# ZhicengShi/mclSTExp

Measured on AMD Instinct MI355X. Metric: training spots/sec (= steps/sec x global batch) at batch 128/GPU, 224px patches, 1000 genes, higher is better.
Workload: dtype bf16; 1 GPU; BASELINE configs[1]: train step, batch 128/GPU, 224x224 patches, 1000 genes, densenet121 image encoder; global_batch=128, parallelism=dp1, backbone_dtype=bf16, infonce=fused, infonce_effective=exact (fused from 1024 pairs), hip_graphs=True, optimizer=Adam(lr=1e-4, wd=1e-3) incl. 2x(65536,G) tables

## Files before the change

include/mclstexp_hip.h:

```cpp
#ifndef MCLSTEXP_HIP_H
#define MCLSTEXP_HIP_H

#include <stddef.h>
#include <stdint.h>

#ifdef __cplusplus
extern "C" {
#endif

#define MCL_ABI_VERSION 13

#define MCL_OK 0
#define MCL_EINVAL (-1)
#define MCL_EUNSUPPORTED (-2)
#define MCL_EWORKSPACE (-3)

typedef void* mcl_stream_t;

int mcl_abi_version(void);
const char* mcl_error_string(int code);

#define MCL_EPI_GELU 1
#define MCL_EPI_GELU_BWD 2
#define MCL_EPI_ACCUM 4
// ... 97 lines not shown

int64_t mcl_infonce_fused_workspace_bytes(int32_t R, int32_t C, int32_t dim);
int mcl_infonce_fused_lse(const void* a, int64_t lda, const void* b, int64_t ldb, int32_t R, int32_t C, int32_t dim,
                          int32_t diag_off, float inv_temp, float* lse, float* diag, void* workspace, int64_t ws_bytes,
                          mcl_stream_t stream);
int mcl_infonce_fused_grad(const void* a, int64_t lda, const void* b, int64_t ldb, int32_t R, int32_t C, int32_t dim,
                           int32_t diag_off, float inv_temp, const float* lse_a, const float* lse_b, float coef, float* dA,
                           void* workspace, int64_t ws_bytes, mcl_stream_t stream);
int mcl_cast_f32_to_bf16(const float* x, int64_t ldx, void* y, int64_t ldy, int64_t rows, int32_t cols,
                         mcl_stream_t stream);

int64_t mcl_gemm_bf16_workspace_floats(int32_t M, int64_t ldc, int32_t ksplit);
int mcl_gemm_bf16(const void* A, int64_t lda, int64_t sAb, const void* B, int64_t ldb, int64_t sBb, void* C, int64_t ldc,
                  int64_t sCb, int32_t M, int32_t N, int32_t K, int32_t batch, int32_t batch2, int64_t sAb2, int64_t sBb2,
                  int64_t sCb2, float alpha, int32_t flags,
                  const float* bias, const void* resid, int64_t ldr, int64_t sRb, const void* aux, int64_t ldaux,
                  void* pre_out, int64_t ldp, int32_t ksplit, float* workspace, int32_t accumulate, mcl_stream_t stream);
int mcl_ln_bf16_fwd(const void* x, int64_t ldx, const float* gamma, const float* beta, void* y, int64_t ldy, float* mean,
                    float* rstd, int64_t rows, int32_t D, float eps, mcl_stream_t stream);
int64_t mcl_colred_workspace_floats(int64_t rows, int32_t D);
int mcl_ln_bf16_bwd(const void* dy, int64_t lddy, const void* x, int64_t ldx, const float* gamma, const float* mean,
                    const float* rstd, const void* dx_add, int64_t ldadd, void* dx, int64_t lddx, float* workspace,
                    float* dgamma, float* dbeta, int32_t accumulate, int64_t rows, int32_t D, mcl_stream_t stream);
int mcl_colsum_bf16(const void* x, int64_t ldx, int64_t rows, int32_t D, float* workspace, float* out, int32_t accumulate,
                    mcl_stream_t stream);
int mcl_softmax_bf16_fwd(void* s, int64_t ld, int64_t rows, int32_t n, mcl_stream_t stream);
int mcl_softmax_bf16_bwd(const void* P, void* dP, int64_t ld, int64_t rows, int32_t n, float scale, mcl_stream_t stream);
int mcl_vit_attn_fwd(const void* qkv, void* o, float* lse, int32_t B, int32_t T, int32_t heads, float scale, mcl_stream_t stream);
int mcl_vit_attn_bwd(const void* qkv, const void* o, const void* dout, const float* lse, float* dsum, void* dqkv, int32_t B,
                     int32_t T, int32_t heads, float scale, mcl_stream_t stream);
int mcl_vit_patchify_tokens(const float* img, int64_t sb, int64_t sc, int64_t sy, int64_t sx, int32_t B, int32_t H, int32_t W,
                            int32_t p, void* out, int32_t lead_zero_row, int32_t out_f32, mcl_stream_t stream);
int mcl_vit_cls_row(const float* cls, const float* pos, void* x, int32_t B, int32_t T, int32_t D, int32_t dtype,
                    mcl_stream_t stream);
int mcl_vit_assemble_f32(const float* tok, const float* cls, const float* pos, float* x, int32_t B, int32_t T, int32_t D,
                         mcl_stream_t stream);
int mcl_vit_tokens_extract(const void* dx, void* dtok, int32_t B, int32_t T, int32_t D, int32_t dtype, mcl_stream_t stream);
int mcl_vit_token_mean_fwd(const void* x, float* feat, int32_t B, int32_t T, int32_t D, int32_t dtype, mcl_stream_t stream);
int mcl_vit_token_mean_bwd(const float* dfeat, void* dx, int32_t B, int32_t T, int32_t D, int32_t dtype, mcl_stream_t stream);
int mcl_vit_pos_grad(const void* dx, float* dpos, float* dcls, int32_t B, int32_t T, int32_t D, int32_t dtype,
                     int32_t accumulate, mcl_stream_t stream);
int mcl_vit_zero_cls_rows(void* dx, int32_t B, int32_t T, int32_t D, int32_t dtype, mcl_stream_t stream);
int mcl_strided4_f32(const float* src, int32_t n0, int32_t n1, int32_t n2, int32_t n3, int64_t a0, int64_t a1, int64_t a2,
                     int64_t a3, void* dst, int64_t d0, int64_t d1, int64_t d2, int64_t d3, int32_t dst_dtype, int32_t accumulate,
                     mcl_stream_t stream);
int mcl_copy_rows(const void* src, int64_t ld_src_bytes, void* dst, int64_t ld_dst_bytes, int64_t rows, int64_t row_bytes,
                  mcl_stream_t stream);
int mcl_weight_rot180(const void* w, void* wf, int32_t Co, int32_t k, int32_t Ci, int32_t dtype, mcl_stream_t stream);
int mcl_vit_patchify(const float* img, int64_t sb, int64_t sc, int64_t sy, int64_t sx, int32_t B, int32_t H, int32_t W,
                     int32_t p, void* out_bf16, mcl_stream_t stream);

int mcl_quant_e4m3_rows(const float* x, int64_t ldx, int32_t rows, int32_t cols, void* q, int64_t ldq, void* scale,
                        int64_t ld_scale, void* deq_bf16, int64_t ldd, mcl_stream_t stream);
int mcl_dequant_e4m3_rows(const void* q, int64_t ldq, const void* scale, int64_t ld_scale, int32_t rows, int32_t cols,
                          void* deq_bf16, int64_t ldd, mcl_stream_t stream);
int64_t mcl_infonce_fp8_workspace_bytes(int32_t R, int32_t C);
int mcl_infonce_fp8_lse(const void* a8, int64_t lda, const void* scale_a, int64_t ld_sa, const void* b8, int64_t ldb,
                        const void* scale_b, int64_t ld_sb, int32_t R, int32_t C, int32_t dim, float inv_temp, float* lse,
                        void* workspace, int64_t ws_bytes, mcl_stream_t stream);
int mcl_infonce_rowdot_bf16(const void* a, int64_t lda, const void* b, int64_t ldb, int32_t R, int32_t C, int32_t dim,
                            int32_t diag_off, float inv_temp, float* diag, mcl_stream_t stream);

int64_t mcl_bn_workspace_floats(int64_t S, int32_t C, int32_t dtype);
int mcl_bn_stats(const void* x, int64_t ld, int64_t S, int32_t C, int32_t dtype, void* copy_out, int64_t ld_out,
                 float* workspace, float eps, float* mean, float* var, float* rstd, mcl_stream_t stream);
int mcl_bn_act_fwd(const void* x, int64_t ldx, int64_t S, int32_t C, int32_t dtype, const float* gamma,
                   const float* beta, const float* mean, const float* rstd, int32_t relu, void* y, int64_t ldy,
                   mcl_stream_t stream);
int mcl_bn_act_bwd(const void* dy, int64_t lddy, const void* x, int64_t ldx, int64_t S, int32_t C, int32_t dtype,
                   const float* gamma, const float* beta, const float* mean, const float* rstd, int32_t relu,
                   float* workspace, float* dgamma, float* dbeta, int32_t accumulate_params, void* dx, int64_t lddx,
                   int32_t accumulate, mcl_stream_t stream);

int64_t mcl_dense_conv1x1_workspace_floats(int64_t S);
int mcl_dense_conv1x1_fwd(const void* x, int64_t ldx, int64_t S, int32_t K, const float* gamma, const float* beta,
                          const float* mean, const float* rstd, const void* W, void* z, int64_t ldz, float* workspace,
                          float eps, float* zmean, float* zvar, float* zrstd, mcl_stream_t stream);

int64_t mcl_dense_conv3x3_workspace_floats(int64_t S);
int mcl_dense_conv3x3_fwd(const void* z, int64_t S, int32_t H, int32_t W, const float* gamma, const float* beta,
                          const float* mean, const float* rstd, const void* W2, void* out, int64_t ldo,
                          float* workspace, float eps, float* ymean, float* yvar, float* yrstd, mcl_stream_t stream);

int64_t mcl_dense_conv3x3_wrw_workspace_floats(int64_t S);
int mcl_dense_conv3x3_wrw_det(const void* dy, int64_t lddy, const void* z, int64_t S, int32_t H, int32_t W,
                              const float* gamma, const float* beta, const float* mean, const float* rstd,
                              float* workspace, float* dW, int32_t accumulate_w, mcl_stream_t stream);

int64_t mcl_dense_bn1_bwd_workspace_floats(int64_t S, int32_t C);
int mcl_dense_bn1_bwd(const void* dz, const void* W1, int32_t C, const void* x, int64_t ldx, int64_t S,
                      const float* gamma, const float* beta, const float* mean, const float* rstd, float* workspace,
                      float* dgamma, float* dbeta, int32_t accumulate_params, void* gbuf, int64_t ldg,
                      mcl_stream_t stream);

int mcl_dense_bn1_dx_window(const void* dz, const void* W1, int32_t C, int32_t c0, int32_t nc, const void* x, int64_t ldx,
                            int64_t S, const float* gamma, const float* beta, const float* mean, const float* rstd,
                            const float* coef, void* gbuf, int64_t ldg, mcl_stream_t stream);
int mcl_dense_bn1_dx_pair(const void* dzA, const void* W1A, int32_t ldwA, const float* gammaA, const float* betaA,
                          const float* coefA, const void* dzB, const void* W1B, const float* gammaB, const float* betaB,
                          const float* coefB, int32_t C, const void* x, int64_t ldx, int64_t S, const float* mean,
                          const float* rstd, void* gbuf, int64_t ldg, mcl_stream_t stream);

int64_t mcl_wrw_workspace_floats(int64_t S, int32_t M, int32_t N);
int mcl_dense_bn1_wrw(const void* dz, const void* W1, int32_t C, const void* x, int64_t ldx, int64_t S,
                      const float* gamma, const float* beta, const float* mean, const float* rstd, float* workspace,
                      float* dW, int32_t accumulate_w, float* dgamma, float* dbeta, int32_t accumulate_params,
                      float* coef_out, mcl_stream_t stream);
int mcl_dense_bn1_dx(const void* dz, const void* W1, int32_t C, const void* x, int64_t ldx, int64_t S,
                     const float* gamma, const float* beta, const float* mean, const float* rstd, const float* coef,
                     void* gbuf, int64_t ldg, mcl_stream_t stream);
int mcl_dense_bn1_dx_sums(const void* dz, const void* W1, int32_t C, const void* x, int64_t ldx, int64_t S,
                          const float* gamma, const float* beta, const float* mean, const float* rstd, float* workspace,
                          float* dgamma, float* dbeta, int32_t accumulate_params, float* kprev, int32_t have_prev, void* gbuf,
                          int64_t ldg, mcl_stream_t stream);
int mcl_dense_bn1_fix(const void* x, int64_t ldx, void* gbuf, int64_t ldg, int64_t S, int32_t c0, int32_t nc,
                      const float* mean, const float* rstd, const float* kacc, mcl_stream_t stream);
int mcl_conv1x1_wrw_det(const void* dz, int64_t ldz, const void* a, int64_t lda, const float* gamma, const float* beta,
                        const float* mean, const float* rstd, float* workspace, float* dW, int32_t accumulate_w,
                        int64_t S, int32_t M, int32_t N, mcl_stream_t stream);

int64_t mcl_dense_conv3x3_bwd_workspace_floats(int64_t S);
int mcl_dense_conv3x3_bwd(const void* dy, int64_t lddy, int64_t S, int32_t H, int32_t W, const void* W2, const void* z,
                          const float* gamma, const float* beta, const float* mean, const float* rstd, float* workspace,
                          float* dgamma, float* dbeta, int32_t accumulate_params, void* g2, void* dz, mcl_stream_t stream);
int mcl_dense_conv3x3_bwd_fix(const void* dy, int64_t lddy, int64_t S, int32_t H, int32_t W, const void* W2, const void* z,
                              const float* gamma, const float* beta, const float* mean, const float* rstd, float* workspace,
                              float* dgamma, float* dbeta, int32_t accumulate_params, void* g2, void* dz, const void* xfix,
                              int64_t ldxf, const float* fmean, const float* frstd, const float* fk, void* dyc,
                              mcl_stream_t stream);

int mcl_avgpool2_nhwc_bf16(const void* x, void* y, int32_t N, int32_t H, int32_t W, int32_t C, int32_t backward,
                           mcl_stream_t stream);
int mcl_maxpool3s2_nhwc_bf16_fwd(const void* x, void* y, void* idx, int32_t N, int32_t H, int32_t W, int32_t C,
                                 mcl_stream_t stream);
int mcl_maxpool3s2_nhwc_bf16_bwd(const void* idx, const void* dy, void* dx, int32_t N, int32_t H, int32_t W, int32_t C,
                                 mcl_stream_t stream);
int mcl_maxpool3s2_nhwc_bf16_bwd_ld(const void* idx, const void* dy, int64_t lddy, void* dx, int32_t N, int32_t H, int32_t W,
                                    int32_t C, mcl_stream_t stream);

int mcl_bn_act_avgpool_fwd(const void* x, int64_t ldx, int32_t N, int32_t H, int32_t W, int32_t C, const float* gamma,
                           const float* beta, const float* mean, const float* rstd, void* y, int64_t ldy,
                           mcl_stream_t stream);
int mcl_bn_act_avgpool_bwd(const void* dp, int64_t lddp, const void* x, int64_t ldx, int32_t N, int32_t H, int32_t W,
                           int32_t C, const float* gamma, const float* beta, const float* mean, const float* rstd,
                           float* workspace, float* dgamma, float* dbeta, int32_t accumulate_params, void* dx,
                           int64_t lddx, mcl_stream_t stream);
int64_t mcl_conv0_workspace_floats(int32_t N, int32_t H, int32_t W);
int mcl_conv0_fwd(const void* x, int32_t N, int32_t H, int32_t W, const void* Wt, void* y, float* workspace, float eps,
                  float* mean, float* var, float* rstd, mcl_stream_t stream);
int64_t mcl_conv0_wrw_workspace_floats(int32_t N, int32_t H, int32_t W);
int mcl_conv0_wrw(const void* x, int32_t N, int32_t H, int32_t W, const void* dy, float* workspace, float* dW,
                  int32_t accumulate_w, mcl_stream_t stream);

int mcl_bn_act_maxpool_fwd(const void* x, int32_t N, int32_t H, int32_t W, int32_t C, const float* gamma,
                           const float* beta, const float* mean, const float* rstd, void* y, void* idx,
                           mcl_stream_t stream);
int mcl_accum_into_f32(float* dst, const void* src, int64_t n, int32_t src_dtype, mcl_stream_t stream);

int mcl_bn_gap_fwd(const void* x, int64_t ldx, int32_t B, int32_t HW, int32_t C, const float* gamma, const float* beta,
                   const float* mean, const float* rstd, float* out, float* xmean, mcl_stream_t stream);
int mcl_bn_gap_bwd(const float* g, const float* xmean, const void* x, int64_t ldx, int32_t B, int32_t HW, int32_t C,
                   const float* gamma, const float* mean, const float* rstd, float* coef, float* dgamma, float* dbeta,
                   int32_t accumulate_params, void* dx, int64_t lddx, mcl_stream_t stream);
int mcl_bn_eval_rstd(int32_t n, const float* const* running_var, float* const* rstd_out, const int32_t* C, const float* eps,
                     mcl_stream_t stream);
int mcl_bn_running_update(int32_t n, float* const* running_mean, float* const* running_var, const float* const* mean,
                          const float* const* var, int64_t* const* num_batches_tracked, const int32_t* C,
                          const float* factor, const float* momentum, mcl_stream_t stream);
int mcl_image_to_bf16_nhwc(const float* x, int64_t sb, int64_t sc, int64_t sy, int64_t sx, int32_t B, int32_t C, int32_t H,
                           int32_t W, void* y, mcl_stream_t stream);
int mcl_fill_zero(void* p, int64_t bytes, mcl_stream_t stream);
int mcl_dropout_fwd(const float* x, float* y, void* mask, int64_t n, float p, uint64_t seed, mcl_stream_t stream);
int mcl_dropout_bwd(const float* dy, const void* mask, float* dx, int64_t n, float p, mcl_stream_t stream);
int mcl_gelu_f32(const float* x, const float* dy, float* out, int64_t n, mcl_stream_t stream);
int mcl_add_f32(const float* a, const float* b, float* y, int64_t n, mcl_stream_t stream);
int mcl_stamp(void* buf, int32_t idx, mcl_stream_t stream);
int mcl_scale2_f32(const float* a, int64_t na, const float* b, int64_t nb, const float* s, float* ya, float* yb,
                   mcl_stream_t stream);

int mcl_im2col_nhwc(const void* x, int64_t ldx, int32_t N, int32_t H, int32_t W, int32_t C, int32_t KH, int32_t KW,
                    int32_t stride, int32_t pad, int32_t dtype, void* cols, mcl_stream_t stream);
int mcl_col2im_nhwc(const void* dcols, int32_t N, int32_t H, int32_t W, int32_t C, int32_t KH, int32_t KW, int32_t stride,
                    int32_t pad, int32_t dtype, void* dx, int64_t lddx, int32_t accumulate, mcl_stream_t stream);
int mcl_maxpool3s2_nhwc_fwd_any(const void* x, void* y, void* idx, int32_t N, int32_t H, int32_t W, int32_t C, int32_t dtype,
                                mcl_stream_t stream);
int mcl_maxpool3s2_nhwc_bwd_any(const void* idx, const void* dy, void* dx, int32_t N, int32_t H, int32_t W, int32_t C,
                                int32_t dtype, mcl_stream_t stream);
int mcl_avgpool2_nhwc_any(const void* x, void* y, int32_t N, int32_t H, int32_t W, int32_t C, int32_t backward, int32_t dtype,
                          mcl_stream_t stream);
int mcl_gap_nhwc_fwd(const void* x, int64_t ldx, int32_t B, int32_t HW, int32_t C, int32_t dtype, float* out,
                     mcl_stream_t stream);
int mcl_gap_nhwc_bwd(const float* g, int32_t B, int32_t HW, int32_t C, int32_t dtype, void* dx, mcl_stream_t stream);
int mcl_add_relu(const void* a, const void* b, void* y, int64_t n, int32_t backward, int32_t dtype, mcl_stream_t stream);

int mcl_dense_block_pack_w1(const void* const* w1_ptrs, void* const* out_ptrs, int32_t L, int32_t C0, mcl_stream_t stream);
int64_t mcl_dense_block_fwd_workspace_bytes(int32_t B, int32_t L);
int mcl_dense_block_fwd(void* buf, int32_t B, int32_t H, int32_t W, int32_t Ct, int32_t C0, int32_t L,
                        const void* const* layer_ptrs, float eps1, float eps2, float* mean, float* var, float* rstd,
                        void* workspace, int32_t* err_flag, uint32_t max_spins, void* stamps, mcl_stream_t stream);

int mcl_dense_block_pack_bwd(const void* const* w1_ptrs, const void* const* w2_ptrs, void* const* w1t_ptrs,
                             void* const* w2t_ptrs, int32_t L, int32_t C0, mcl_stream_t stream);
int64_t mcl_dense_block_bwd_workspace_bytes(int32_t B, int32_t L);
int mcl_dense_block_bwd(const void* buf, void* gbuf, int32_t B, int32_t H, int32_t W, int32_t Ct, int32_t C0, int32_t L,
                        const void* const* layer_ptrs, const float* mean, const float* rstd, void* workspace,
                        int32_t* err_flag, uint32_t max_spins, void* stamps, mcl_stream_t stream);

int mcl_adam_step(float* p, const float* g, float* m, float* v, int64_t n, double lr, double beta1, double beta2,
                  double eps, double weight_decay, double bc1, double bc2, mcl_stream_t stream);
int mcl_adam_table_step(float* p, float* m, float* v, int32_t n_rows, int32_t cols, const int32_t* row_slot,
                        const float* row_grad, int64_t ld_rg, double lr, double beta1, double beta2, double eps,
                        double weight_decay, double bc1, double bc2, mcl_stream_t stream);
// ... 286 lines not shown
```

mclstexp_amd/_lib.py:

```python
from __future__ import annotations

import ctypes as C
import os
from typing import Optional

import torch

_HERE = os.path.dirname(os.path.abspath(__file__))
LIB_PATH = os.environ.get("MCL_LIB_PATH") or os.path.join(_HERE, "libmclstexp_hip.so")
ABI_VERSION = 13

_lib: Optional[C.CDLL] = None

c_f = C.c_float
c_d = C.c_double
c_i = C.c_int32
c_l = C.c_int64
c_p = C.c_void_p


class c_s(C.c_void_p):
    """mcl_stream_t: the trailing stream slot of an entry point.  ``call`` fills it in with torch's current stream."""


# ... 63 lines not shown
    "mcl_infonce_dlogits": [c_p, c_l, c_p, c_p, c_i, c_i, c_i, c_i, c_f, c_p, c_l, c_s],
    "mcl_infonce_fused_workspace_bytes": [c_i, c_i, c_i],
    "mcl_infonce_fused_lse": [c_p, c_l, c_p, c_l, c_i, c_i, c_i, c_i, c_f, c_p, c_p, c_p, c_l, c_s],
    "mcl_infonce_fused_grad": [c_p, c_l, c_p, c_l, c_i, c_i, c_i, c_i, c_f, c_p, c_p, c_f, c_p, c_p, c_l, c_s],
    "mcl_cast_f32_to_bf16": [c_p, c_l, c_p, c_l, c_l, c_i, c_s],
    "mcl_infonce_loss_mean": [c_p, c_l, c_p, c_p, c_i, c_f, c_p, c_s],
    "mcl_adam_step_dev_shadow": [c_p, c_p, c_p, c_p, c_l, c_p, c_p, c_s],
    "mcl_bn_gap_fwd": [c_p, c_l, c_i, c_i, c_i, c_p, c_p, c_p, c_p, c_p, c_p, c_s],
    "mcl_bn_gap_bwd": [c_p, c_p, c_p, c_l, c_i, c_i, c_i, c_p, c_p, c_p, c_p, c_p, c_p, c_i, c_p, c_l, c_s],
    "mcl_bn_running_update": [c_i, c_p, c_p, c_p, c_p, c_p, c_p, c_p, c_p, c_s],
    "mcl_bn_eval_rstd": [c_i, c_p, c_p, c_p, c_p, c_s],
    "mcl_image_to_bf16_nhwc": [c_p, c_l, c_l, c_l, c_l, c_i, c_i, c_i, c_i, c_p, c_s],
    "mcl_fill_zero": [c_p, c_l, c_s],
    "mcl_stamp": [c_p, c_i, c_s],
    "mcl_dropout_fwd": [c_p, c_p, c_p, c_l, c_f, C.c_uint64, c_s],
    "mcl_dropout_bwd": [c_p, c_p, c_p, c_l, c_f, c_s],
    "mcl_gelu_f32": [c_p, c_p, c_p, c_l, c_s],
    "mcl_add_f32": [c_p, c_p, c_p, c_l, c_s],
    "mcl_im2col_nhwc": [c_p, c_l, c_i, c_i, c_i, c_i, c_i, c_i, c_i, c_i, c_i, c_p, c_s],
    "mcl_col2im_nhwc": [c_p, c_i, c_i, c_i, c_i, c_i, c_i, c_i, c_i, c_i, c_p, c_l, c_i, c_s],
    "mcl_maxpool3s2_nhwc_fwd_any": [c_p, c_p, c_p, c_i, c_i, c_i, c_i, c_i, c_s],
    "mcl_maxpool3s2_nhwc_bwd_any": [c_p, c_p, c_p, c_i, c_i, c_i, c_i, c_i, c_s],
    "mcl_avgpool2_nhwc_any": [c_p, c_p, c_i, c_i, c_i, c_i, c_i, c_i, c_s],
    "mcl_gap_nhwc_fwd": [c_p, c_l, c_i, c_i, c_i, c_i, c_p, c_s],
    "mcl_gap_nhwc_bwd": [c_p, c_i, c_i, c_i, c_i, c_p, c_s],
    "mcl_add_relu": [c_p, c_p, c_p, c_l, c_i, c_i, c_s],
    "mcl_scale2_f32": [c_p, c_l, c_p, c_l, c_p, c_p, c_p, c_s],
    "mcl_maxpool3s2_nhwc_bf16_bwd_ld": [c_p, c_p, c_l, c_p, c_i, c_i, c_i, c_i, c_s],
    "mcl_gemm_bf16_workspace_floats": [c_i, c_l, c_i],
    "mcl_gemm_bf16": [c_p, c_l, c_l, c_p, c_l, c_l, c_p, c_l, c_l, c_i, c_i, c_i, c_i, c_i, c_l, c_l, c_l, c_f, c_i, c_p,
                      c_p, c_l, c_l, c_p, c_l, c_p, c_l, c_i, c_p, c_i, c_s],
    "mcl_ln_bf16_fwd": [c_p, c_l, c_p, c_p, c_p, c_l, c_p, c_p, c_l, c_i, c_f, c_s],
    "mcl_colred_workspace_floats": [c_l, c_i],
    "mcl_ln_bf16_bwd": [c_p, c_l, c_p, c_l, c_p, c_p, c_p, c_p, c_l, c_p, c_l, c_p, c_p, c_p, c_i, c_l, c_i, c_s],
    "mcl_colsum_bf16": [c_p, c_l, c_l, c_i, c_p, c_p, c_i, c_s],
    "mcl_softmax_bf16_fwd": [c_p, c_l, c_l, c_i, c_s],
    "mcl_softmax_bf16_bwd": [c_p, c_p, c_l, c_l, c_i, c_f, c_s],
    "mcl_vit_patchify": [c_p, c_l, c_l, c_l, c_l, c_i, c_i, c_i, c_i, c_p, c_s],
    "mcl_vit_patchify_tokens": [c_p, c_l, c_l, c_l, c_l, c_i, c_i, c_i, c_i, c_p, c_i, c_i, c_s],
    "mcl_vit_cls_row": [c_p, c_p, c_p, c_i, c_i, c_i, c_i, c_s],
    "mcl_vit_assemble_f32": [c_p, c_p, c_p, c_p, c_i, c_i, c_i, c_s],
    "mcl_vit_tokens_extract": [c_p, c_p, c_i, c_i, c_i, c_i, c_s],
    "mcl_vit_token_mean_fwd": [c_p, c_p, c_i, c_i, c_i, c_i, c_s],
    "mcl_vit_token_mean_bwd": [c_p, c_p, c_i, c_i, c_i, c_i, c_s],
    "mcl_vit_pos_grad": [c_p, c_p, c_p, c_i, c_i, c_i, c_i, c_i, c_s],
    "mcl_vit_zero_cls_rows": [c_p, c_i, c_i, c_i, c_i, c_s],
    "mcl_strided4_f32": [c_p, c_i, c_i, c_i, c_i, c_l, c_l, c_l, c_l, c_p, c_l, c_l, c_l, c_l, c_i, c_i, c_s],
    "mcl_copy_rows": [c_p, c_l, c_p, c_l, c_l, c_l, c_s],
    "mcl_weight_rot180": [c_p, c_p, c_i, c_i, c_i, c_i, c_s],
    "mcl_vit_attn_fwd": [c_p, c_p, c_p, c_i, c_i, c_i, c_f, c_s],
    "mcl_vit_attn_bwd": [c_p, c_p, c_p, c_p, c_p, c_p, c_i, c_i, c_i, c_f, c_s],
    "mcl_quant_e4m3_rows": [c_p, c_l, c_i, c_i, c_p, c_l, c_p, c_l, c_p, c_l, c_s],
    "mcl_dequant_e4m3_rows": [c_p, c_l, c_p, c_l, c_i, c_i, c_p, c_l, c_s],
    "mcl_infonce_fp8_workspace_bytes": [c_i, c_i],
    "mcl_infonce_fp8_lse": [c_p, c_l, c_p, c_l, c_p, c_l, c_p, c_l, c_i, c_i, c_i, c_f, c_p, c_p, c_l, c_s],
    "mcl_infonce_rowdot_bf16": [c_p, c_l, c_p, c_l, c_i, c_i, c_i, c_i, c_f, c_p, c_s],
    "mcl_bn_workspace_floats": [c_l, c_i, c_i],
    "mcl_bn_stats": [c_p, c_l, c_l, c_i, c_i, c_p, c_l, c_p, c_f, c_p, c_p, c_p, c_s],
    "mcl_bn_act_fwd": [c_p, c_l, c_l, c_i, c_i, c_p, c_p, c_p, c_p, c_i, c_p, c_l, c_s],
    "mcl_bn_act_bwd": [c_p, c_l, c_p, c_l, c_l, c_i, c_i, c_p, c_p, c_p, c_p, c_i, c_p, c_p, c_p, c_i, c_p, c_l, c_i, c_s],
    "mcl_dense_conv1x1_workspace_floats": [c_l],
    "mcl_dense_conv1x1_fwd": [c_p, c_l, c_l, c_i, c_p, c_p, c_p, c_p, c_p, c_p, c_l, c_p, c_f, c_p, c_p, c_p, c_s],
    "mcl_dense_conv3x3_workspace_floats": [c_l],
    "mcl_dense_bn1_bwd_workspace_floats": [c_l, c_i],
    "mcl_dense_conv3x3_bwd_workspace_floats": [c_l],
    "mcl_avgpool2_nhwc_bf16": [c_p, c_p, c_i, c_i, c_i, c_i, c_i, c_s],
    "mcl_maxpool3s2_nhwc_bf16_fwd": [c_p, c_p, c_p, c_i, c_i, c_i, c_i, c_s],
    "mcl_maxpool3s2_nhwc_bf16_bwd": [c_p, c_p, c_p, c_i, c_i, c_i, c_i, c_s],
    "mcl_dense_conv3x3_bwd": [c_p, c_l, c_l, c_i, c_i, c_p, c_p, c_p, c_p, c_p, c_p, c_p, c_p, c_p, c_i, c_p, c_p, c_s],
    "mcl_dense_conv3x3_bwd_fix": [c_p, c_l, c_l, c_i, c_i, c_p, c_p, c_p, c_p, c_p, c_p, c_p, c_p, c_p, c_i, c_p, c_p, c_p,
                                  c_l, c_p, c_p, c_p, c_p, c_s],
    "mcl_dense_bn1_bwd": [c_p, c_p, c_i, c_p, c_l, c_l, c_p, c_p, c_p, c_p, c_p, c_p, c_p, c_i, c_p, c_l, c_s],
    "mcl_dense_conv3x3_wrw_workspace_floats": [c_l],
    "mcl_dense_conv3x3_wrw_det": [c_p, c_l, c_p, c_l, c_i, c_i, c_p, c_p, c_p, c_p, c_p, c_p, c_i, c_s],
    "mcl_wrw_workspace_floats": [c_l, c_i, c_i],
    "mcl_dense_bn1_wrw": [c_p, c_p, c_i, c_p, c_l, c_l, c_p, c_p, c_p, c_p, c_p, c_p, c_i, c_p, c_p, c_i, c_p, c_s],
    "mcl_dense_bn1_dx_window": [c_p, c_p, c_i, c_i, c_i, c_p, c_l, c_l, c_p, c_p, c_p, c_p, c_p, c_p, c_l, c_s],
    "mcl_dense_bn1_dx_pair": [c_p, c_p, c_i, c_p, c_p, c_p, c_p, c_p, c_p, c_p, c_p, c_i, c_p, c_l, c_l, c_p, c_p, c_p, c_l, c_s],
    "mcl_dense_bn1_dx": [c_p, c_p, c_i, c_p, c_l, c_l, c_p, c_p, c_p, c_p, c_p, c_p, c_l, c_s],
    "mcl_dense_bn1_dx_sums": [c_p, c_p, c_i, c_p, c_l, c_l, c_p, c_p, c_p, c_p, c_p, c_p, c_p, c_i, c_p, c_i, c_p, c_l, c_s],
    "mcl_dense_bn1_fix": [c_p, c_l, c_p, c_l, c_l, c_i, c_i, c_p, c_p, c_p, c_s],
    "mcl_conv1x1_wrw_det": [c_p, c_l, c_p, c_l, c_p, c_p, c_p, c_p, c_p, c_p, c_i, c_l, c_i, c_i, c_s],
    "mcl_dense_conv3x3_fwd": [c_p, c_l, c_i, c_i, c_p, c_p, c_p, c_p, c_p, c_p, c_l, c_p, c_f, c_p, c_p, c_p, c_s],
    "mcl_accum_into_f32": [c_p, c_p, c_l, c_i, c_s],
    "mcl_adam_step": [c_p, c_p, c_p, c_p, c_l, c_d, c_d, c_d, c_d, c_d, c_d, c_d, c_s],
    "mcl_adam_table_step": [c_p, c_p, c_p, c_i, c_i, c_p, c_p, c_l, c_d, c_d, c_d, c_d, c_d, c_d, c_d, c_s],
    "mcl_adam_consts_update": [c_p, c_p, c_p, c_s],
    "mcl_adam_step_dev": [c_p, c_p, c_p, c_p, c_l, c_p, c_s],
    "mcl_adam_table_step_dev": [c_p, c_p, c_p, c_i, c_i, c_p, c_p, c_l, c_p, c_s],
    "mcl_row_slot_update": [c_p, c_p, c_i, c_i, c_s],
    "mcl_dense_block_fwd_workspace_bytes": [c_i, c_i],
    "mcl_dense_block_pack_w1": [c_p, c_p, c_i, c_i, c_s],
    "mcl_dense_block_pack_bwd": [c_p, c_p, c_p, c_p, c_i, c_i, c_s],
    "mcl_dense_block_bwd_workspace_bytes": [c_i, c_i],
    "mcl_dense_block_bwd": [c_p, c_p, c_i, c_i, c_i, c_i, c_i, c_i, c_p, c_p, c_p, c_p, c_p, C.c_uint32, c_p, c_s],
    "mcl_dense_block_fwd": [c_p, c_i, c_i, c_i, c_i, c_i, c_i, c_p, c_f, c_f, c_p, c_p, c_p, c_p, c_p, C.c_uint32, c_p, c_s],
    "mcl_adam_consts_update_hist": [c_p, c_p, c_p, c_p, c_i, c_s],
    "mcl_adam_table_lazy": [c_p, c_p, c_p, c_p, c_p, c_p, c_p, c_p, c_i, c_i, c_p, c_p, c_p, c_i, c_p, c_p, c_l, c_p, c_p, c_i,
                            c_s],
    "mcl_bn_act_avgpool_fwd": [c_p, c_l, c_i, c_i, c_i, c_i, c_p, c_p, c_p, c_p, c_p, c_l, c_s],
    "mcl_bn_act_avgpool_bwd": [c_p, c_l, c_p, c_l, c_i, c_i, c_i, c_i, c_p, c_p, c_p, c_p, c_p, c_p, c_p, c_i, c_p, c_l,
                               c_s],
    "mcl_conv0_workspace_floats": [c_i, c_i, c_i],
    "mcl_conv0_fwd": [c_p, c_i, c_i, c_i, c_p, c_p, c_p, c_f, c_p, c_p, c_p, c_s],
    "mcl_conv0_wrw_workspace_floats": [c_i, c_i, c_i],
    "mcl_conv0_wrw": [c_p, c_i, c_i, c_i, c_p, c_p, c_p, c_i, c_s],
    "mcl_bn_act_maxpool_fwd": [c_p, c_i, c_i, c_i, c_i, c_p, c_p, c_p, c_p, c_p, c_p, c_s],
    "mcl_patch_gather": [c_p, c_i, c_i, c_p, c_i, c_i, c_p, c_f, c_p, c_p, c_s],
    "mcl_her2st_train_patches": [c_p, c_i, c_i, c_p, c_i, c_i, c_p, c_f, c_p, c_p, c_s],
    "mcl_log_library_size_normalize": [c_p, c_l, c_p, c_l, c_i, c_i, c_f, c_s],
    "mcl_l2_normalize_rows": [c_p, c_l, c_p, c_l, c_i, c_i, c_s],
    "mcl_topk_rows_max_k": [],
    "mcl_topk_rows": [c_p, c_l, c_i, c_i, c_i, c_p, c_p, c_s],
    "mcl_topk_rows_indexed": [c_p, c_l, c_p, c_l, c_i, c_i, c_i, c_p, c_p, c_p, c_s],
    "mcl_knn_weighted_average": [c_p, c_l, c_p, c_l, c_p, c_l, c_p, c_i, c_i, c_i, c_i, c_i, c_p, c_p, c_s],
    "mcl_expr_metrics": [c_p, c_l, c_i, c_p, c_l, c_i, c_p, c_i, c_i, c_i, c_p, c_p, c_p, c_p, c_p, c_s],
    "mcl_pearson_pvalue": [c_p, c_p, c_i, c_i, c_p, c_p, c_s],
    "mcl_gene_rank": [c_p, c_p, c_i, c_i, c_i, c_p, c_p, c_p, c_p, c_p, c_p, c_s],
    "mcl_knn_combine": [c_p, c_l, c_p, c_l, c_p, c_l, c_p, c_i, c_i, c_i, c_i, c_i, c_p, c_p, c_s],
    "mcl_cell_pearson": [c_p, c_l, c_i, c_p, c_l, c_i, c_l, c_i, c_p, c_s],
    "mcl_bleep_summary": [c_p, c_l, c_i, c_p, c_i, c_i, c_i, c_p, c_p, c_p, c_i, c_p, c_p, c_p, c_p, c_p, c_s],
    "mcl_corr_from_gram": [c_p, c_i, c_p, c_s],
    "mcl_pca_gram": [c_p, c_l, c_i, c_p, c_i, c_i, c_i, c_p, c_p, c_p, c_s],
    "mcl_pca_project": [c_p, c_l, c_i, c_p, c_i, c_i, c_i, c_i, c_p, c_p, c_p, c_p, c_p, c_p, c_p, c_s],
    "mcl_kmeans": [c_p, c_l, c_p, c_i, c_l, c_i, c_p, c_i, c_i, c_p, C.c_uint64, c_i, c_d, c_i, c_p, c_p, c_p, c_p, c_p, c_p,
                   c_p, c_p, c_p, c_p, c_p, c_s],
    "mcl_cluster_scores": [c_p, c_p, c_p, c_i, c_i, c_p, c_s],
    "mcl_hvg_stats": [c_p, c_p, c_p, c_p, c_p, c_i, c_p, c_i, c_i, c_i, c_i, c_p, c_p, c_p, c_p, c_p, c_p, c_p, c_p, c_p, c_s],
    "mcl_hvg_pool": [c_p, c_i, c_i, c_p, c_i, c_p, c_p, c_s],
    "mcl_expression_matrices": [c_p, c_p, c_p, c_p, c_p, c_i, c_p, c_i, c_i, c_i, c_f, c_p, c_s],
    "mcl_harmony_workspace_doubles": [c_i, c_i, c_i, c_i],
    "mcl_harmony_normalize": [c_p, c_l, c_i, c_i, c_i, c_i, c_p, c_p, c_s],
    "mcl_harmony_centroids": [c_p, c_p, c_p, c_i, c_i, c_i, c_i, c_i, c_p, c_p, c_s],
    "mcl_harmony_dist": [c_p, c_p, c_i, c_i, c_i, c_i, c_p, c_s],
    "mcl_harmony_softmax": [c_p, c_i, c_i, c_d, c_i, c_p, c_s],
    "mcl_harmony_moments": [c_p, c_p, c_i, c_i, c_i, c_p, c_p, c_p, c_s],
    "mcl_harmony_update_block": [c_p, c_p, c_p, c_p, c_i, c_i, c_i, c_i, c_i, c_i, c_p, c_p, c_p, c_p, c_s],
    "mcl_harmony_objective": [c_p, c_p, c_p, c_p, c_p, c_p, c_i, c_i, c_i, c_d, c_p, c_p, c_s],
    "mcl_harmony_ridge": [c_p, c_p, c_p, c_i, c_i, c_i, c_p, c_s],
    "mcl_harmony_apply": [c_p, c_p, c_p, c_p, c_i, c_i, c_i, c_i, c_p, c_s],
    "mcl_harmony_lloyd": [c_p, c_i, c_i, c_i, c_p, c_i, c_p, c_p, c_p, c_p, c_p, c_s],
    "mcl_tsne_workspace_doubles": [c_i, c_i],
    "mcl_tsne_affinities": [c_p, c_l, c_i, c_i, c_p, c_p, c_i, c_i, c_i, c_i, c_l, c_d, c_i, c_p, c_p, c_p, c_s],
    "mcl_tsne_gradient": [c_p, c_p, c_p, c_p, c_i, c_i, c_i, c_i, c_l, c_p, c_i, c_p, c_p, c_p, c_s],
    "mcl_tsne_update": [c_p, c_p, c_i, c_i, c_i, c_i, c_p, c_p, c_p, c_p, c_p, c_s],
    "mcl_knn_workspace_bytes": [c_i, c_i],
    "mcl_knn_exact": [c_p, c_l, c_i, c_i, c_p, c_i, c_i, c_i, c_i, c_i, c_p, c_p, c_s],
    "mcl_knn_smooth": [c_p, c_p, c_i, c_i, c_i, c_i, c_i, c_p, c_p, c_p, c_s],
    "mcl_knn_connectivities": [c_p, c_p, c_p, c_p, c_p, c_i, c_i, c_i, c_i, c_i, c_d, c_i, c_p, c_p, c_p, c_p, c_l, c_p, c_p,
                               c_s],
    "mcl_umap_workspace_bytes": [c_l, c_i],
    "mcl_umap_prepare": [c_p, c_p, c_p, c_i, c_l, c_l, c_i, c_i, c_p, c_p, c_s],
    "mcl_umap_init": [c_i, c_p, c_l, c_i, c_i, c_p, c_i, c_i, c_i, c_i, C.c_uint64, c_p, c_s],
    "mcl_umap_epochs": [c_i, c_i, c_p, c_p, c_p, c_p, c_p, c_i, c_i, c_i, c_i, c_l, c_i, c_d, c_d, c_d, c_d, c_i, C.c_uint64,
                        c_p, c_p, c_p, c_p, c_s],
    "mcl_leiden_workspace_bytes": [c_l, c_l, c_i, c_i],
    "mcl_leiden_init": [c_p, c_p, c_p, c_p, c_p, c_i, c_i, c_i, c_l, c_d, c_p, c_p, c_p, c_p],
    "mcl_leiden_move_sweeps": [c_i, c_i, c_i, c_i, c_i, c_p, c_p, c_p, c_p, c_i, c_i, c_i, c_l, c_d, c_p, c_p],
    "mcl_leiden_refine_rounds": [c_i, c_i, c_i, c_i, c_i, c_i, c_p, c_p, c_p, c_p, c_i, c_i, c_i, c_l, c_d, c_p, c_p],
    "mcl_leiden_aggregate": [c_i, c_i, c_i, c_p, c_p, c_p, c_p, c_i, c_i, c_i, c_l, c_d, c_p, c_p],
    "mcl_leiden_finish": [c_i, c_i, c_p, c_p, c_p, c_p, c_p, c_i, c_i, c_i, c_l, c_p, c_p, c_p, c_p, c_p],
    "mcl_sym_eig_workspace_bytes": [c_i, c_i, c_l, c_i],
    "mcl_sym_eig_top": [c_p, c_p, c_p, c_i, c_i, c_l, c_i, c_i, c_p, c_p, c_p, c_p, c_p, c_p],
    "mcl_marker_workspace_bytes": [c_l, c_l, c_i, c_i],
    "mcl_marker_stats": [c_p, c_l, c_i, c_p, c_p, c_p, c_i, c_l, c_i, c_i, c_i, c_l, c_p, c_p, c_p, c_p, c_p, c_p, c_p, c_p,
                         c_p, c_p, c_p, c_p, c_p],
# ... 197 lines not shown
```

mclstexp_amd/csrc/dense_bwd.hip:

```cpp
#include "common.h"
#include <stdlib.h>

namespace {

constexpr int TN = 128, TK = 128;

__device__ __forceinline__ uint4 keep4(bool keep, const uint4 v) {
  return make_uint4(keep ? v.x : 0u, keep ? v.y : 0u, keep ? v.z : 0u, keep ? v.w : 0u);
}

template <int MODE, int TMv>
__global__ __launch_bounds__(256, (TMv == 64 && MODE != 2 ? 3 : 2)) void bn1_bwd_kernel(const bf16_t* __restrict__ dz, const bf16_t* __restrict__ W1,
                                                         int K , int ldw ,
                                                         const bf16_t* __restrict__ x, long long ldx, long long S,
                                                         const float* __restrict__ gamma,
                                                         const float* __restrict__ beta,
                                                         const float* __restrict__ mean,
                                                         const float* __restrict__ rstd,
                                                         const float* __restrict__ coef ,
                                                         bf16_t* gbuf, long long ldg,
                                                         float2* __restrict__ partial , int nrt) {
  __shared__ __attribute__((aligned(16))) unsigned char lds[TK * 256 + TMv * 256 + 2048];
  const int tid = threadIdx.x, lane = tid & 63, wave = tid >> 6;
  const int h = lane >> 5, l31 = lane & 31;
// ... 404 lines not shown
  for (int o = 32; o > 0; o >>= 1) {
    a += __shfl_xor(a, o, 64);
    b += __shfl_xor(b, o, 64);
  }
  if (lane == 0) {
    red[0][wave] = a;
    red[1][wave] = b;
  }
  __syncthreads();
  if (threadIdx.x != 0) return;
  a = (red[0][0] + red[0][1]) + (red[0][2] + red[0][3]);
  b = (red[1][0] + red[1][1]) + (red[1][2] + red[1][3]);
  if (accumulate_params) {
    dbeta[c] += (float)a;
    dgamma[c] += (float)b;
  } else {
    dbeta[c] = (float)a;
    dgamma[c] = (float)b;
  }
  if (kacc != nullptr) {
    const double scv = (double)gamma[c] * (double)rstd[c];
    kacc[2 * c] = (float)(scv * a / (double)S);
    kacc[2 * c + 1] = (float)(scv * b / (double)S);
    return;
  }
  coef[2 * c] = (float)(a / (double)S);
  coef[2 * c + 1] = (float)(b / (double)S);
}

__global__ __launch_bounds__(256) void bn1_fix_kernel(const bf16_t* __restrict__ x, long long ldx, bf16_t* __restrict__ gbuf,
                                                      long long ldg, long long S, int c0, int nc,
                                                      const float* __restrict__ mean, const float* __restrict__ rstd,
                                                      const float* __restrict__ kacc) {
  const int cpr = nc >> 3;
  const long long n = S * cpr;
  const long long i0 = (long long)blockIdx.x * 256 + threadIdx.x, istride = (long long)gridDim.x * 256;
  const bool fixed = (istride % cpr) == 0;
  uint4 xv = make_uint4(0u, 0u, 0u, 0u), gv = xv;
  if (i0 < n) {
    const long long row = i0 / cpr;
    const int c = c0 + (int)(i0 - row * cpr) * 8;
    xv = *reinterpret_cast<const uint4*>(x + row * ldx + c);
    gv = *reinterpret_cast<const uint4*>(gbuf + row * ldg + c);
  }
  float kav[8], kbv[8];
  auto consts = [&](int c) {
#pragma unroll
    for (int e = 0; e < 8; ++e) {
      const float k1 = kacc[2 * (c + e)], k2 = kacc[2 * (c + e) + 1];
      kav[e] = k2 * rstd[c + e];
      kbv[e] = fmaf(-kav[e], mean[c + e], k1);
    }
  };
  if (i0 < n) consts(c0 + (int)(i0 % cpr) * 8);
  for (long long i = i0; i < n; i += istride) {
    const long long row = i / cpr;
    const int c = c0 + (int)(i - row * cpr) * 8;
    if (i != i0) {
      xv = *reinterpret_cast<const uint4*>(x + row * ldx + c);
      gv = *reinterpret_cast<const uint4*>(gbuf + row * ldg + c);
      if (!fixed) consts(c);
    }
    const unsigned xw[4] = {xv.x, xv.y, xv.z, xv.w};
    unsigned gw[4] = {gv.x, gv.y, gv.z, gv.w};
#pragma unroll
    for (int u = 0; u < 4; ++u) {
      float o[2];
#pragma unroll
      for (int e = 0; e < 2; ++e) {
        const float ka = kav[2 * u + e], kb = kbv[2 * u + e];
        const float xf = e ? __uint_as_float(xw[u] & 0xFFFF0000u) : __uint_as_float(xw[u] << 16);
        const float gf = e ? __uint_as_float(gw[u] & 0xFFFF0000u) : __uint_as_float(gw[u] << 16);
        o[e] = gf - fmaf(ka, xf, kb);
      }
      const f32x2 pv = {o[0], o[1]};
      gw[u] = __builtin_bit_cast(unsigned, __builtin_convertvector(pv, bf16x2_t));
    }
    *reinterpret_cast<uint4*>(gbuf + row * ldg + c) = make_uint4(gw[0], gw[1], gw[2], gw[3]);
  }
}

constexpr int C3I = 128, C3O = 32, T3B = 128;

__global__ __launch_bounds__(256, 1) void conv3x3_bwd_kernel(const bf16_t* __restrict__ dy, long long lddy, long long S,
                                                             int H, int W, const bf16_t* __restrict__ W2,
                                                             const bf16_t* __restrict__ z,
                                                             const float* __restrict__ gamma,
                                                             const float* __restrict__ beta,
                                                             const float* __restrict__ mean,
                                                             const float* __restrict__ rstd, bf16_t* __restrict__ g2,
                                                             float2* __restrict__ partial, int ntile,
                                                             const bf16_t* __restrict__ xfix, long long ldxf,
                                                             const float* __restrict__ fmean,
                                                             const float* __restrict__ frstd,
                                                             const float* __restrict__ fk, bf16_t* __restrict__ dyc) {
  extern __shared__ __attribute__((aligned(16))) unsigned char lds[];
  const int tid = threadIdx.x, lane = tid & 63, wave = tid >> 6;
  const int h = lane >> 5, l31 = lane & 31;
  const int nrow = T3B + 2 * W + 2;
  bf16_t* zt = reinterpret_cast<bf16_t*>(lds);
  unsigned char* slab = lds + T3B * 256;
  const int zero_off = T3B * 256 + nrow * 64;
  const int Si = (int)S;

  uint4 zr[8];
  auto load_z_tile = [&](int tile) {
    const int p0 = tile * T3B;
#pragma unroll
    for (int i = 0; i < 8; ++i) {
      const int p = p0 + (tid >> 4) + 16 * i;
      zr[i] = p < Si ? *reinterpret_cast<const uint4*>(z + (long long)p * C3I + (tid & 15) * 8) : make_uint4(0u, 0u, 0u, 0u);
    }
  };
  if ((int)blockIdx.x < ntile) load_z_tile(blockIdx.x);
  bf16x8 breg[18];
#pragma unroll
  for (int i = 0; i < 18; ++i) {
    const int tap = i >> 1, co0 = 16 * (i & 1) + 8 * h;
#pragma unroll
    for (int j = 0; j < 8; ++j)
      breg[i][j] = (short)W2[((long long)(co0 + j) * 9 + tap) * C3I + 32 * wave + l31];
  }
  const int c = 32 * wave + l31;
  const float mu = mean[c], rs = rstd[c];
  const float sc = gamma[c] * rs, sh = fmaf(-mu, sc, beta[c]);
  int abase[18];
#pragma unroll
  for (int i = 0; i < 18; ++i) {
    const int tap = i >> 1, ky = tap / 3, kx = tap % 3;
    const int row = l31 + (2 - ky) * W + (2 - kx);
    abase[i] = T3B * 256 + row * 64 + (((2 * (i & 1) + h) ^ ((row >> 2) & 3)) << 4);
  }
  if (tid < 4) *reinterpret_cast<uint4*>(lds + zero_off + tid * 16) = make_uint4(0u, 0u, 0u, 0u);
  float fka[8], fkb[8];
  if (xfix != nullptr) {
#pragma unroll
    for (int e = 0; e < 8; ++e) {
      const int cf = (tid & 3) * 8 + e;
      const float k1 = fk[2 * cf], k2 = fk[2 * cf + 1];
      fka[e] = k2 * frstd[cf];
      fkb[e] = fmaf(-fka[e], fmean[cf], k1);
    }
  }

  for (int tile = blockIdx.x; tile < ntile; tile += gridDim.x) {
    const int p0 = tile * T3B;
    if (tile != (int)blockIdx.x) load_z_tile(tile);
    __syncthreads();
    for (int q = tid; q < nrow * 4; q += 256) {
      const int j = q >> 2, ch = q & 3;
      const int p = p0 - (W + 1) + j;
      uint4 v = make_uint4(0u, 0u, 0u, 0u);
      if (p >= 0 && p < Si) {
        v = *reinterpret_cast<const uint4*>(dy + (long long)p * lddy + ch * 8);
        if (xfix != nullptr) {
          const uint4 xv = *reinterpret_cast<const uint4*>(xfix + (long long)p * ldxf + ch * 8);
          const unsigned xw[4] = {xv.x, xv.y, xv.z, xv.w};
          unsigned gw[4] = {v.x, v.y, v.z, v.w};
#pragma unroll
          for (int u = 0; u < 4; ++u) {
            const float o_lo = __uint_as_float(gw[u] << 16) - fmaf(fka[2 * u], __uint_as_float(xw[u] << 16), fkb[2 * u]);
            const float o_hi = __uint_as_float(gw[u] & 0xFFFF0000u) -
                               fmaf(fka[2 * u + 1], __uint_as_float(xw[u] & 0xFFFF0000u), fkb[2 * u + 1]);
            const f32x2 pv = {o_lo, o_hi};
            gw[u] = __builtin_bit_cast(unsigned, __builtin_convertvector(pv, bf16x2_t));
          }
          v = make_uint4(gw[0], gw[1], gw[2], gw[3]);
          if (dyc != nullptr && j >= W + 1 && j < W + 1 + T3B) *reinterpret_cast<uint4*>(dyc + (long long)p * C3O + ch * 8) = v;
        }
      }
      *reinterpret_cast<uint4*>(slab + j * 64 + ((ch ^ ((j >> 2) & 3)) << 4)) = v;
    }
#pragma unroll
    for (int i = 0; i < 8; ++i)
      *reinterpret_cast<uint4*>(zt + ((tid >> 4) + 16 * i) * C3I + (tid & 15) * 8) = zr[i];
    unsigned vmask[4];
#pragma unroll
    for (int mb = 0; mb < 4; ++mb) {
      const int p = p0 + mb * 32 + l31;
      const int x = p % W, y = (p / W) % H;
      unsigned m = 0;
      if (p < Si) {
#pragma unroll
        for (int ky = 0; ky < 3; ++ky)
#pragma unroll
          for (int kx = 0; kx < 3; ++kx) {
            const int yy = y + 1 - ky, xx = x + 1 - kx;
            if (yy >= 0 && yy < H && xx >= 0 && xx < W) m |= 1u << (ky * 3 + kx);
          }
      }
      vmask[mb] = m;
    }
    f32x16 acc[4];
#pragma unroll
    for (int mb = 0; mb < 4; ++mb)
#pragma unroll
      for (int r = 0; r < 16; ++r) acc[mb][r] = 0.0f;
    __syncthreads();

#pragma unroll
    for (int i = 0; i < 18; ++i) {
#pragma unroll
      for (int mb = 0; mb < 4; ++mb) {
        const int off = ((vmask[mb] >> (i >> 1)) & 1u) ? abase[i] + mb * 2048 : zero_off;
        const bf16x8 a = *reinterpret_cast<const bf16x8*>(lds + off);
        acc[mb] = __builtin_amdgcn_mfma_f32_32x32x16_bf16(a, breg[i], acc[mb], 0, 0, 0);
      }
    }
    const int nvalid = min(T3B, Si - p0);
    float s1 = 0.0f, s2 = 0.0f;
#pragma unroll
    for (int mb = 0; mb < 4; ++mb)
#pragma unroll
      for (int r = 0; r < 16; ++r) {
        const int px = mb * 32 + (r & 3) + 8 * (r >> 2) + 4 * h;
        const float zv = bf2f(zt[px * C3I + c]);
        const float gi = fmaf(zv, sc, sh) > 0.0f ? acc[mb][r] : 0.0f;
        const bf16_t gb = f2bf(gi);
        if (px < nvalid) {
          const float gr_ = bf2f(gb);
          s1 += gr_;
          s2 = fmaf(gr_, (zv - mu) * rs, s2);
        }
        zt[px * C3I + c] = gb;
      }
    s1 += __shfl_xor(s1, 32, 64);
    s2 += __shfl_xor(s2, 32, 64);
    if (h == 0) partial[(long long)c * ntile + tile] = make_float2(s1, s2);
    __syncthreads();
#pragma unroll
    for (int i = 0; i < 8; ++i) {
      const int r = (tid >> 4) + 16 * i;
      const int p = p0 + r;
      if (p < Si)
        *reinterpret_cast<uint4*>(g2 + (long long)p * C3I + (tid & 15) * 8) =
            *reinterpret_cast<const uint4*>(zt + r * C3I + (tid & 15) * 8);
    }
  }
}

constexpr int BR_NWAVE = 8;
constexpr int BR_SLOT = 34 * 64;
constexpr int BR_RING = 4 * BR_SLOT;

__device__ __forceinline__ void br_swap8(unsigned (&w)[8]) {
#pragma unroll
  for (int g = 0; g < 2; ++g)
#pragma unroll
    for (int d = 0; d < 2; ++d) {
      const u32x2 r = __builtin_amdgcn_permlane32_swap(w[4 * g + d], w[4 * g + 2 + d], false, false);
      w[4 * g + d] = r[0];
      w[4 * g + 2 + d] = r[1];
    }
}

template <bool K0, bool K2>
__device__ __forceinline__ void br_row_mfma(const unsigned char* __restrict__ ring, int jo, const int (&foff)[3][2],
                                            const bf16x8 (&breg)[18], f32x16& acc) {
// ... 326 lines not shown
  if (nb > 2048) nb = 2048;
  hipLaunchKernelGGL(bn1_fix_kernel, dim3((int)nb), dim3(256), 0, mcl_stream(stream), (const bf16_t*)x, (long long)ldx,
                     (bf16_t*)gbuf, (long long)ldg, (long long)S, c0, nc, mean, rstd, kacc);
  MCL_CHECK_LAUNCH();
  return MCL_OK;
}

namespace {
int bn1_dx_impl(const void* dz, const void* W1, int32_t C, int32_t ldw, const void* x, int64_t ldx, int64_t S, const float* gamma,
                const float* beta, const float* mean, const float* rstd, const float* coef, void* gbuf, int64_t ldg,
                mcl_stream_t stream) {
  if (!dz || !W1 || !x || !gamma || !beta || !mean || !rstd || !coef || !gbuf || S <= 0 || C <= 0 || ldw < C) return MCL_EINVAL;
  if ((C % 8) || (ldw % 8) || (ldx % 8) || (ldg % 8) || (reinterpret_cast<uintptr_t>(dz) & 15u) ||
      (reinterpret_cast<uintptr_t>(W1) & 15u) || (reinterpret_cast<uintptr_t>(x) & 15u) ||
      (reinterpret_cast<uintptr_t>(gbuf) & 15u))
    return MCL_EUNSUPPORTED;
  const int nrt = (int)((S + 63) / 64), nct = (C + TN - 1) / TN;
  const int gcap = S >= 50000 ? 512 : 768;
  int gx = (gcap + nct - 1) / nct;
  if (gx > nrt) gx = nrt;
  hipLaunchKernelGGL((bn1_bwd_kernel<1, 64>), dim3(gx, nct), dim3(256), 0, mcl_stream(stream), (const bf16_t*)dz,
                     (const bf16_t*)W1, C, ldw, (const bf16_t*)x, (long long)ldx, (long long)S, gamma, beta, mean, rstd, coef,
                     (bf16_t*)gbuf, (long long)ldg, (float2*)nullptr, nrt);
  MCL_CHECK_LAUNCH();
  return MCL_OK;
}
}

extern "C" int mcl_dense_bn1_dx(const void* dz, const void* W1, int32_t C, const void* x, int64_t ldx, int64_t S,
                                const float* gamma, const float* beta, const float* mean, const float* rstd,
                                const float* coef, void* gbuf, int64_t ldg, mcl_stream_t stream) {
  MCL_CLEAR_ERROR();
  return bn1_dx_impl(dz, W1, C, C, x, ldx, S, gamma, beta, mean, rstd, coef, gbuf, ldg, stream);
}

extern "C" int mcl_dense_bn1_dx_window(const void* dz, const void* W1, int32_t C, int32_t c0, int32_t nc, const void* x,
                                       int64_t ldx, int64_t S, const float* gamma, const float* beta, const float* mean,
                                       const float* rstd, const float* coef, void* gbuf, int64_t ldg, mcl_stream_t stream) {
  MCL_CLEAR_ERROR();
  if (c0 < 0 || nc <= 0 || c0 + nc > C || (c0 % 8)) return MCL_EINVAL;
  if (!dz || !W1 || !x || !gamma || !beta || !mean || !rstd || !coef || !gbuf) return MCL_EINVAL;
  return bn1_dx_impl(dz, (const bf16_t*)W1 + c0, nc, C, (const bf16_t*)x + c0, ldx, S, gamma + c0, beta + c0, mean + c0, rstd + c0,
                     coef + 2 * c0, (bf16_t*)gbuf + c0, ldg, stream);
}

extern "C" int mcl_dense_bn1_dx_pair(const void* dzA, const void* W1A, int32_t ldwA, const float* gammaA, const float* betaA,
                                     const float* coefA, const void* dzB, const void* W1B, const float* gammaB,
                                     const float* betaB, const float* coefB, int32_t C, const void* x, int64_t ldx, int64_t S,
                                     const float* mean, const float* rstd, void* gbuf, int64_t ldg, mcl_stream_t stream) {
  MCL_CLEAR_ERROR();
  if (!dzA || !W1A || !gammaA || !betaA || !coefA || !dzB || !W1B || !gammaB || !betaB || !coefB || !x || !mean || !rstd || !gbuf ||
      S <= 0 || C <= 0 || ldwA < C)
    return MCL_EINVAL;
  if ((C % 8) || (ldwA % 8) || (ldx % 8) || (ldg % 8) || (reinterpret_cast<uintptr_t>(dzA) & 15u) ||
      (reinterpret_cast<uintptr_t>(dzB) & 15u) || (reinterpret_cast<uintptr_t>(W1A) & 15u) ||
      (reinterpret_cast<uintptr_t>(W1B) & 15u) || (reinterpret_cast<uintptr_t>(x) & 15u) ||
      (reinterpret_cast<uintptr_t>(gbuf) & 15u))
    return MCL_EUNSUPPORTED;
  static mcl_device_once attr_once;
  if (auto guard = attr_once.first())
    (void)hipFuncSetAttribute(reinterpret_cast<const void*>(bn1_dx_pair_kernel), hipFuncAttributeMaxDynamicSharedMemorySize,
                              (int)PAIR_LDS);
  const int nrt = (int)((S + 63) / 64), nct = (C + TN - 1) / TN;
  const int gcap = 512;
  int gx = (gcap + nct - 1) / nct;
  if (gx > nrt) gx = nrt;
  hipLaunchKernelGGL(bn1_dx_pair_kernel, dim3(gx, nct), dim3(256), PAIR_LDS, mcl_stream(stream), (const bf16_t*)dzA,
                     (const bf16_t*)W1A, ldwA, gammaA, betaA, coefA, (const bf16_t*)dzB, (const bf16_t*)W1B, gammaB, betaB, coefB, C,
                     (const bf16_t*)x, (long long)ldx, (long long)S, mean, rstd, (bf16_t*)gbuf, (long long)ldg, nrt);
  MCL_CHECK_LAUNCH();
  return MCL_OK;
}

extern "C" int64_t mcl_dense_conv3x3_bwd_workspace_floats(int64_t S) {
  if (S <= 0) return -1;
  const int64_t flat = (S + T3B - 1) / T3B, rows = S / 32 + 8;
  return (flat > rows ? flat : rows) * 2 * (int64_t)C3I + 2 * (int64_t)C3I;
}

namespace {
int conv3x3_bwd_impl(const void* dy, int64_t lddy, int64_t S, int32_t H, int32_t W, const void* W2, const void* z,
                     const float* gamma, const float* beta, const float* mean, const float* rstd, float* workspace,
                     float* dgamma, float* dbeta, int32_t accumulate_params, void* g2, void* dz, const void* xfix,
                     int64_t ldxf, const float* fmean, const float* frstd, const float* fk, void* dyc, mcl_stream_t stream) {
  MCL_CLEAR_ERROR();
  if (!dy || !W2 || !z || !gamma || !beta || !mean || !rstd || !workspace || !dgamma || !dbeta || !g2 || !dz || S <= 0 ||
      H <= 0 || W <= 0)
    return MCL_EINVAL;
  if ((S % ((int64_t)H * W)) || S > 0x7fff0000LL || W > 150 || (lddy % 8) || lddy < C3O ||
      (reinterpret_cast<uintptr_t>(dy) & 15u) || (reinterpret_cast<uintptr_t>(z) & 15u) ||
      (reinterpret_cast<uintptr_t>(g2) & 15u) || (reinterpret_cast<uintptr_t>(dz) & 15u))
    return MCL_EUNSUPPORTED;
  if (xfix != nullptr) {
    if (!fmean || !frstd || !fk || !dyc) return MCL_EINVAL;
    if (bwd_rows_applicable(S, H, W) || (ldxf % 8) || (reinterpret_cast<uintptr_t>(xfix) & 15u) ||
        (reinterpret_cast<uintptr_t>(dyc) & 15u))
      return MCL_EUNSUPPORTED;
  }
  hipStream_t st = mcl_stream(stream);
  float2* part = reinterpret_cast<float2*>(workspace);
  float* coef;
  if (bwd_rows_applicable(S, H, W)) {
    const BwdRowsPlan p = bwd_rows_plan(S, H, W);
    coef = workspace + (int64_t)p.nsu * 2 * C3I;
    static mcl_device_once attr_once;
    if (auto attr_guard = attr_once.first()) {
      (void)hipFuncSetAttribute(reinterpret_cast<const void*>(conv3x3_bwd_rows_kernel),
                                hipFuncAttributeMaxDynamicSharedMemorySize, 160 * 1024);
    }
    hipLaunchKernelGGL(conv3x3_bwd_rows_kernel, dim3(p.grid), dim3(64 * BR_NWAVE), (size_t)BR_NWAVE * BR_RING + 1024, st,
                       (const bf16_t*)dy, (long long)lddy, p.nimg, H, W, (const bf16_t*)W2, (const bf16_t*)z, gamma, beta,
                       mean, rstd, (bf16_t*)g2, part, p.nsu, p.rc, p.nchunk, p.nstrip);
    hipLaunchKernelGGL(bn1_bwd_finalize_kernel, dim3(C3I), dim3(256), 0, st, (const float2*)part, p.nsu, C3I,
                       (long long)S, dgamma, dbeta, coef, accumulate_params);
  } else {
    const int ntile = (int)((S + T3B - 1) / T3B);
    coef = workspace + (int64_t)ntile * 2 * C3I;
    const size_t lds_bytes = (size_t)T3B * 256 + (size_t)(T3B + 2 * W + 2) * 64 + 64;
    const int gcap = S >= 50000 ? 512 : 768;
    hipLaunchKernelGGL(conv3x3_bwd_kernel, dim3(ntile < gcap ? ntile : gcap), dim3(256), lds_bytes, st, (const bf16_t*)dy,
                       (long long)lddy, (long long)S, H, W, (const bf16_t*)W2, (const bf16_t*)z, gamma, beta, mean, rstd,
                       (bf16_t*)g2, part, ntile, (const bf16_t*)xfix, (long long)ldxf, fmean, frstd, fk, (bf16_t*)dyc);
    hipLaunchKernelGGL(bn1_bwd_finalize_kernel, dim3(C3I), dim3(256), 0, st, (const float2*)part, ntile, C3I,
                       (long long)S, dgamma, dbeta, coef, accumulate_params);
  }
  const long long n_chunks = S * (C3I / 8);
  long long blocks = (n_chunks + 255) / 256;
  if (blocks > 2048) blocks = 2048;
  hipLaunchKernelGGL(bn2_dz_kernel, dim3((unsigned)blocks), dim3(256), 0, st, (const bf16_t*)g2, (const bf16_t*)z,
                     n_chunks, gamma, mean, rstd, (const float*)coef, (bf16_t*)dz);
  MCL_CHECK_LAUNCH();
  return MCL_OK;
}
}

extern "C" int mcl_dense_conv3x3_bwd(const void* dy, int64_t lddy, int64_t S, int32_t H, int32_t W, const void* W2,
                                     const void* z, const float* gamma, const float* beta, const float* mean,
                                     const float* rstd, float* workspace, float* dgamma, float* dbeta,
                                     int32_t accumulate_params, void* g2, void* dz, mcl_stream_t stream) {
  return conv3x3_bwd_impl(dy, lddy, S, H, W, W2, z, gamma, beta, mean, rstd, workspace, dgamma, dbeta, accumulate_params, g2,
                          dz, nullptr, 0, nullptr, nullptr, nullptr, nullptr, stream);
}

extern "C" int mcl_dense_conv3x3_bwd_fix(const void* dy, int64_t lddy, int64_t S, int32_t H, int32_t W, const void* W2,
                                         const void* z, const float* gamma, const float* beta, const float* mean,
                                         const float* rstd, float* workspace, float* dgamma, float* dbeta,
                                         int32_t accumulate_params, void* g2, void* dz, const void* xfix, int64_t ldxf,
                                         const float* fmean, const float* frstd, const float* fk, void* dyc,
                                         mcl_stream_t stream) {
  if (!xfix) return MCL_EINVAL;
  return conv3x3_bwd_impl(dy, lddy, S, H, W, W2, z, gamma, beta, mean, rstd, workspace, dgamma, dbeta, accumulate_params, g2,
                          dz, xfix, ldxf, fmean, frstd, fk, dyc, stream);
}
```

mclstexp_amd/csrc/dense_conv.hip:

```cpp
#include "common.h"

namespace {

constexpr int BN = 128;
constexpr int BK = 64;

template <int WM, int RW = 64, int DEPTH = 1>
__global__ __launch_bounds__(128 * WM) void conv1x1_fwd_kernel(const bf16_t* __restrict__ x, long long ldx, long long S,
                                                               int K, const float* __restrict__ gamma,
                                                               const float* __restrict__ beta,
                                                               const float* __restrict__ mean,
                                                               const float* __restrict__ rstd,
                                                               const bf16_t* __restrict__ W, bf16_t* __restrict__ z,
                                                               long long ldz, float2* __restrict__ partial, int nblk) {
  constexpr int BM = RW * WM, NT = 128 * WM;
  constexpr int RI = RW / 32;
  constexpr int NA = (BM * 8) / NT;
  constexpr int A_B = BM * 128, B_B = BN * 128, STAGE_B = A_B + B_B;
  constexpr int NB = (BN * 8) / NT;
  constexpr int NBUF = DEPTH == 0 ? 1 : 2, NSET = DEPTH == 0 ? 1 : DEPTH;
  __shared__ __attribute__((aligned(16))) unsigned char lds[NBUF * STAGE_B + 2 * 1024 * 4];
  float* tab = reinterpret_cast<float*>(lds + NBUF * STAGE_B);

  const int tid = threadIdx.x, lane = tid & 63, wave = tid >> 6;
// ... 240 lines not shown
    red[0][wave] = sum;
    red[1][wave] = q;
  }
  __syncthreads();
  if (threadIdx.x != 0) return;
  sum = (red[0][0] + red[0][1]) + (red[0][2] + red[0][3]);
  q = (red[1][0] + red[1][1]) + (red[1][2] + red[1][3]);
  const double n = (double)S, m = sum / n;
  double v = (q - sum * sum / n) / n;
  if (v < 0.0) v = 0.0;
  mean[c] = (float)m;
  var[c] = (float)v;
  rstd[c] = (float)(1.0 / sqrt(v + (double)eps));
}

inline int pick_wm(long long S) { return S >= 32768 ? 2 : 1; }

}

extern "C" int64_t mcl_dense_conv1x1_workspace_floats(int64_t S) {
  if (S <= 0) return -1;
  const int bm = 64 * pick_wm(S);
  return ((S + bm - 1) / bm) * BN * 2;
}

extern "C" int mcl_dense_conv1x1_fwd(const void* x, int64_t ldx, int64_t S, int32_t K, const float* gamma,
                                     const float* beta, const float* mean, const float* rstd, const void* W, void* z,
                                     int64_t ldz, float* workspace, float eps, float* zmean, float* zvar,
                                     float* zrstd, mcl_stream_t stream) {
  MCL_CLEAR_ERROR();
  if (!x || !gamma || !beta || !mean || !rstd || !W || !z || !workspace || S <= 0 || K <= 0) return MCL_EINVAL;
  const bool want_stats = zmean || zvar || zrstd;
  if (want_stats && (!zmean || !zvar || !zrstd)) return MCL_EINVAL;
  if ((K % 8) || K > 1024 || (ldx % 8) || (ldz % 8) || ldz < BN || S * ldx * 2 >= 0xFFFFF000LL  ||
      (reinterpret_cast<uintptr_t>(x) & 15u) ||
      (reinterpret_cast<uintptr_t>(W) & 15u) || (reinterpret_cast<uintptr_t>(z) & 15u))
    return MCL_EUNSUPPORTED;
  const int wm = pick_wm(S);
  const int bm = 64 * wm;
  const int nblk = (int)((S + bm - 1) / bm);
  hipStream_t st = mcl_stream(stream);
  float2* part = reinterpret_cast<float2*>(workspace);
#define MCL_LAUNCH(WMV, RWV, DPV)                                                                                    \
  hipLaunchKernelGGL((conv1x1_fwd_kernel<WMV, RWV, DPV>), dim3(nblk), dim3(128 * WMV), 0, st, (const bf16_t*)x,      \
                     (long long)ldx, (long long)S, K, gamma, beta, mean, rstd, (const bf16_t*)W, (bf16_t*)z,          \
                     (long long)ldz, part, nblk)
  if (wm == 2) MCL_LAUNCH(2, 64, 0);
  else MCL_LAUNCH(2, 32, 4);
#undef MCL_LAUNCH
  if (want_stats)
    hipLaunchKernelGGL(tile_stats_finalize_kernel, dim3(BN), dim3(256), 0, st, (const float2*)part, nblk, BN,
                       (long long)S, bm, eps, zmean, zvar, zrstd);
  MCL_CHECK_LAUNCH();
  return MCL_OK;
}

constexpr int C3_IN = 128, C3_OUT = 32, T3 = 128;

constexpr int SLAB_NB = 8;
template <int NB>
__device__ __forceinline__ void stage_slab(unsigned char* lds, const bf16_t* __restrict__ z, int p0, long long S,
                                           int W, int nrow, int tid, const float (&sc)[8], const float (&sh)[8]) {
  const int cc = tid & 15;
  for (int jb = tid >> 4; jb < nrow; jb += 16 * NB) {
    uint4 v[NB];
    bool ok[NB];
#pragma unroll
    for (int i = 0; i < NB; ++i) {
      const int j = jb + 16 * i;
      const int p = p0 - (W + 1) + j;
      ok[i] = j < nrow && p >= 0 && p < (int)S;
      v[i] = ok[i] ? *reinterpret_cast<const uint4*>(z + (long long)p * C3_IN + cc * 8) : make_uint4(0u, 0u, 0u, 0u);
    }
#pragma unroll
    for (int i = 0; i < NB; ++i) {
      const int j = jb + 16 * i;
      if (j < nrow)
        *reinterpret_cast<uint4*>(lds + j * 256 + ((cc ^ (j & 15)) << 4)) =
            ok[i] ? bn_relu_chunk(v[i], sc, sh) : make_uint4(0u, 0u, 0u, 0u);
    }
  }
}

__global__ __launch_bounds__(256, 2) void conv3x3_fwd_kernel(const bf16_t* __restrict__ z, long long S, int H, int W,
                                                             const float* __restrict__ gamma,
                                                             const float* __restrict__ beta,
                                                             const float* __restrict__ mean,
                                                             const float* __restrict__ rstd,
                                                             const bf16_t* __restrict__ W2, bf16_t* __restrict__ out,
                                                             long long ldo, float2* __restrict__ partial, int ntile) {
  extern __shared__ __attribute__((aligned(16))) unsigned char lds[];
  const int tid = threadIdx.x, lane = tid & 63, wave = tid >> 6;
  const int h = lane >> 5, l31 = lane & 31;
  const int nrow = T3 + 2 * W + 2;
  unsigned char* zero_row = lds + nrow * 256;
  const int Si = (int)S;

  bf16x8 breg[18];
#pragma unroll
  for (int i = 0; i < 18; ++i) {
    const int kidx = 18 * wave + i;
    breg[i] = *reinterpret_cast<const bf16x8*>(W2 + ((long long)l31 * 9 + (kidx >> 3)) * C3_IN + 16 * (kidx & 7) + 8 * h);
  }
  float sc[8], sh[8];
  {
    const int cc = tid & 15;
#pragma unroll
    for (int i = 0; i < 8; ++i) {
      const int c = cc * 8 + i;
      sc[i] = gamma[c] * rstd[c];
      sh[i] = fmaf(-mean[c], sc[i], beta[c]);
    }
  }
  int abase[18], tapk[18];
#pragma unroll
  for (int i = 0; i < 18; ++i) {
    const int kidx = 18 * wave + i, tap = kidx >> 3, kk = kidx & 7;
    const int row = l31 + (tap / 3) * W + (tap % 3);
    abase[i] = row * 256 + (((2 * kk + h) ^ (row & 15)) << 4);
    tapk[i] = tap;
  }
  for (int tile = blockIdx.x; tile < ntile; tile += gridDim.x) {
  const int p0 = tile * T3;
  __syncthreads();

  stage_slab<SLAB_NB>(lds, z, p0, S, W, nrow, tid, sc, sh);
  if (tid < 16) *reinterpret_cast<uint4*>(zero_row + tid * 16) = make_uint4(0u, 0u, 0u, 0u);

  unsigned vmask[4];
#pragma unroll
  for (int mb = 0; mb < 4; ++mb) {
    const int p = p0 + mb * 32 + l31;
    const int x = p % W, y = (p / W) % H;
    unsigned m = 0;
    if (p < Si) {
#pragma unroll
      for (int ky = 0; ky < 3; ++ky)
#pragma unroll
        for (int kx = 0; kx < 3; ++kx) {
          const int yy = y + ky - 1, xx = x + kx - 1;
          if (yy >= 0 && yy < H && xx >= 0 && xx < W) m |= 1u << (ky * 3 + kx);
        }
    }
    vmask[mb] = m;
  }
  f32x16 acc[4];
#pragma unroll
  for (int mb = 0; mb < 4; ++mb)
#pragma unroll
    for (int r = 0; r < 16; ++r) acc[mb][r] = 0.0f;
  __syncthreads();

  const int zero_off = nrow * 256;
#pragma unroll
  for (int i = 0; i < 18; ++i) {
#pragma unroll
    for (int mb = 0; mb < 4; ++mb) {
      const int off = ((vmask[mb] >> tapk[i]) & 1u) ? abase[i] + mb * 8192 : zero_off;
      const bf16x8 a = *reinterpret_cast<const bf16x8*>(lds + off);
      acc[mb] = __builtin_amdgcn_mfma_f32_32x32x16_bf16(a, breg[i], acc[mb], 0, 0, 0);
    }
  }
  __syncthreads();
  float* red = reinterpret_cast<float*>(lds);
#pragma unroll
  for (int mb = 0; mb < 4; ++mb)
#pragma unroll
    for (int r = 0; r < 16; ++r) {
      const int px = mb * 32 + (r & 3) + 8 * (r >> 2) + 4 * h;
      red[(wave * T3 + px) * C3_OUT + l31] = acc[mb][r];
    }
  __syncthreads();
  const int px = tid >> 1, c0 = (tid & 1) * 16;
  const long long p = (long long)p0 + px;
  float v[16];
#pragma unroll
  for (int q = 0; q < 4; ++q) {
    float4 s = *reinterpret_cast<const float4*>(red + px * C3_OUT + c0 + 4 * q);
#pragma unroll
    for (int w = 1; w < 4; ++w) {
      const float4 t = *reinterpret_cast<const float4*>(red + (w * T3 + px) * C3_OUT + c0 + 4 * q);
      s.x += t.x; s.y += t.y; s.z += t.z; s.w += t.w;
    }
    v[4 * q] = s.x; v[4 * q + 1] = s.y; v[4 * q + 2] = s.z; v[4 * q + 3] = s.w;
  }
  unsigned pk[8];
#pragma unroll
  for (int q = 0; q < 8; ++q) pk[q] = pack_bf16(v[2 * q], v[2 * q + 1]);
  if (p < S) {
    *reinterpret_cast<uint4*>(out + p * ldo + c0) = make_uint4(pk[0], pk[1], pk[2], pk[3]);
    *reinterpret_cast<uint4*>(out + p * ldo + c0 + 8) = make_uint4(pk[4], pk[5], pk[6], pk[7]);
  }
  __syncthreads();
  float* rv = reinterpret_cast<float*>(lds);
  float* grp = rv + T3 * C3_OUT;
#pragma unroll
  for (int q = 0; q < 8; ++q) {
    rv[px * C3_OUT + c0 + 2 * q] = bf_lo(pk[q]);
    rv[px * C3_OUT + c0 + 2 * q + 1] = bf_hi(pk[q]);
  }
  __syncthreads();
  {
    const int c = tid & 31, g = tid >> 5;
    const float ks = rv[c];
    const int nvalid = min(T3, Si - p0);
    float s1 = 0.0f, s2 = 0.0f;
#pragma unroll
    for (int q = 0; q < 16; ++q) {
      const int pp = g * 16 + q;
      if (pp < nvalid) {
        const float dlt = rv[pp * C3_OUT + c] - ks;
        s1 += dlt;
        s2 = fmaf(dlt, dlt, s2);
      }
    }
    grp[(g * 32 + c) * 2] = s1;
    grp[(g * 32 + c) * 2 + 1] = s2;
    __syncthreads();
    if (tid < 32) {
      float a = 0.0f, b = 0.0f;
#pragma unroll
      for (int gg = 0; gg < 8; ++gg) {
        a += grp[(gg * 32 + tid) * 2];
        b += grp[(gg * 32 + tid) * 2 + 1];
      }
      const float n = (float)nvalid;
      partial[(long long)tid * ntile + tile] = make_float2(fmaf(n, rv[tid], a), b - a * a / n);
    }
  }
  }
}

extern "C" int64_t mcl_dense_conv3x3_workspace_floats(int64_t S) {
  if (S <= 0) return -1;
  const int64_t flat = ((S + T3 - 1) / T3) * C3_OUT * 2, rows = mcl_conv3x3_rows_workspace_floats(S);
  return flat > rows ? flat : rows;
}

extern "C" int mcl_dense_conv3x3_fwd(const void* z, int64_t S, int32_t H, int32_t W, const float* gamma,
                                     const float* beta, const float* mean, const float* rstd, const void* W2, void* out,
                                     int64_t ldo, float* workspace, float eps, float* ymean, float* yvar, float* yrstd,
                                     mcl_stream_t stream) {
  MCL_CLEAR_ERROR();
  if (!z || !gamma || !beta || !mean || !rstd || !W2 || !out || !workspace || S <= 0 || H <= 0 || W <= 0)
    return MCL_EINVAL;
  const bool want_stats = ymean || yvar || yrstd;
  if (want_stats && (!ymean || !yvar || !yrstd)) return MCL_EINVAL;
  if ((S % ((int64_t)H * W)) || S > 0x7fff0000LL || W > 150 || (ldo % 8) || ldo < C3_OUT || (reinterpret_cast<uintptr_t>(z) & 15u) ||
      (reinterpret_cast<uintptr_t>(W2) & 15u) || (reinterpret_cast<uintptr_t>(out) & 15u))
    return MCL_EUNSUPPORTED;
  if (mcl_conv3x3_rows_applicable(S, H, W)) {
    const int rc = mcl_launch_conv3x3_fwd_rows(z, S, H, W, gamma, beta, mean, rstd, W2, out, ldo, workspace, eps, ymean,
                                               yvar, yrstd, mcl_stream(stream));
    if (rc != 0) return rc;
    MCL_CHECK_LAUNCH();
    return MCL_OK;
  }
  const int ntile = (int)((S + T3 - 1) / T3);
  size_t lds_bytes = (size_t)(T3 + 2 * W + 2) * 256 + 256;
  if (lds_bytes < 4 * T3 * C3_OUT * 4) lds_bytes = 4 * T3 * C3_OUT * 4;
  hipStream_t st = mcl_stream(stream);
  static mcl_device_once attr_once;
  if (auto attr_guard = attr_once.first()) {
    (void)hipFuncSetAttribute(reinterpret_cast<const void*>(conv3x3_fwd_kernel),
                              hipFuncAttributeMaxDynamicSharedMemorySize, 112 * 1024);
  }
  float2* part = reinterpret_cast<float2*>(workspace);
  hipLaunchKernelGGL(conv3x3_fwd_kernel, dim3(ntile < 512 ? ntile : 512), dim3(256), lds_bytes, st, (const bf16_t*)z, (long long)S, H, W,
                     gamma, beta, mean, rstd, (const bf16_t*)W2, (bf16_t*)out, (long long)ldo, part, ntile);
  if (want_stats)
    hipLaunchKernelGGL(tile_stats_finalize_kernel, dim3(C3_OUT), dim3(256), 0, st, (const float2*)part, ntile,
                       C3_OUT, (long long)S, T3, eps, ymean, yvar, yrstd);
  MCL_CHECK_LAUNCH();
  return MCL_OK;
}

namespace {

__device__ __forceinline__ int w3k_swz(int row) { return ((row & 3) << 2) | ((row >> 2) & 3); }

constexpr int W3K_ROWS = T3 + 2;
constexpr int W3K_LDS = W3K_ROWS * 256 + 3 * T3 * 64;

__global__ __launch_bounds__(256, 2) void conv3x3_wrw_ky_kernel(const bf16_t* __restrict__ dy, long long lddy,
                                                                const bf16_t* __restrict__ z, long long S, int H, int W,
                                                                const float* __restrict__ gamma,
                                                                const float* __restrict__ beta,
                                                                const float* __restrict__ mean,
                                                                const float* __restrict__ rstd, int ntile, int G,
                                                                float* __restrict__ wpart) {
  __shared__ __attribute__((aligned(16))) unsigned char lds[W3K_LDS];
  const int tid = threadIdx.x, lane = tid & 63, wave = tid >> 6;
  const int h = lane >> 5, l31 = lane & 31;
  const int xcd = blockIdx.x & 7, slot = blockIdx.x >> 3;
  const int ky = slot % 3, g = (slot / 3) * 8 + xcd;
  if (g >= G) return;
  unsigned char* zt = lds;
  unsigned char* dyt = lds + W3K_ROWS * 256;
  const int Si = (int)S;

  const int cc = tid & 15, rz = tid >> 4;
  const int rd = tid >> 1, cd = (tid & 1) * 2;
  float sc[8], sh[8];
#pragma unroll
  for (int i = 0; i < 8; ++i) {
    const int c = cc * 8 + i;
    sc[i] = gamma[c] * rstd[c];
    sh[i] = fmaf(-mean[c], sc[i], beta[c]);
  }
  f32x16 acc[3];
#pragma unroll
  for (int b = 0; b < 3; ++b)
#pragma unroll
    for (int r = 0; r < 16; ++r) acc[b][r] = 0.0f;

  const int i15 = lane & 15, q = i15 >> 2, jj = i15 & 3;
  const int half16 = 16 * ((lane >> 4) & 1);
  const int byte = (jj & 1) * 8;
  int bz_lo[3], bz_hi[3];
#pragma unroll
  for (int kx = 0; kx < 3; ++kx) {
    const int chunk = wave * 4 + ((half16 + jj * 4) >> 3);
    const int r0 = 8 * h + q + kx, r1 = r0 + 4;
    bz_lo[kx] = r0 * 256 + ((chunk ^ w3k_swz(r0)) << 4) + byte;
    bz_hi[kx] = r1 * 256 + ((chunk ^ w3k_swz(r1)) << 4) + byte;
  }
  const int dchunk = (half16 + jj * 4) >> 3;

  auto fetch = [&](uint4 (&zv)[9], uint4 (&dv)[2], int tile) {
    const int p0 = tile * T3;
    const int qs = p0 + (ky - 1) * W - 1;
#pragma unroll
    for (int i = 0; i < 9; ++i) {
      const int j = rz + 16 * i;
      const int p = qs + j;
      zv[i] = (tile < ntile && j < W3K_ROWS && p >= 0 && p < Si)
                  ? *reinterpret_cast<const uint4*>(z + (long long)p * C3_IN + cc * 8)
                  : make_uint4(0u, 0u, 0u, 0u);
    }
    const int p = p0 + rd;
#pragma unroll
    for (int u = 0; u < 2; ++u)
      dv[u] = (tile < ntile && p < Si) ? *reinterpret_cast<const uint4*>(dy + (long long)p * lddy + (cd + u) * 8)
                                       : make_uint4(0u, 0u, 0u, 0u);
  };
  auto stage = [&](const uint4 (&zv)[9], const uint4 (&dv)[2], int tile) {
    const int p0 = tile * T3;
    const int qs = p0 + (ky - 1) * W - 1;
#pragma unroll
    for (int i = 0; i < 9; ++i) {
      const int j = rz + 16 * i;
      if (j < W3K_ROWS) {
        const int p = qs + j;
        const bool ok = p >= 0 && p < Si;
        *reinterpret_cast<uint4*>(zt + j * 256 + ((cc ^ w3k_swz(j)) << 4)) =
            ok ? bn_relu_chunk(zv[i], sc, sh) : make_uint4(0u, 0u, 0u, 0u);
      }
// ... 435 lines not shown
```

mclstexp_amd/densenet_fused.py:

```python
from __future__ import annotations

import contextlib
import os
from typing import List, NamedTuple, Optional, Tuple

import torch
import torch.nn.functional as F
from torch import nn

from ._lib import call, current_stream

Tensor = torch.Tensor
CL = torch.channels_last
_ws_cache = {}

_fallbacks: dict = {}


def fallback_counts() -> dict:
    return dict(_fallbacks)


def reset_fallbacks() -> None:
    _fallbacks.clear()
# ... 252 lines not shown
    else:
        dg = torch.empty(C, device=x.device, dtype=torch.float32)
        db = torch.empty(C, device=x.device, dtype=torch.float32)
    call("mcl_dense_bn1_bwd", dz, w16, C, px, ldx, S, g1, b1, mean, rstd, ws, dg, db, into_param_grads, pg, ldg)
    return (None, None) if into_param_grads else (dg, db)


def dense_bn1_dx_sums(dz: Tensor, w16: Tensor, x: Tensor, g1: Tensor, b1: Tensor, mean: Tensor, rstd: Tensor, gbuf: Tensor,
                      kprev: Tensor, have_prev: bool, into_param_grads: bool) -> Tuple[Optional[Tensor], Optional[Tensor]]:
    px, S, C, ldx = _rows(x)
    pg, S2, C2, ldg = _rows(gbuf)
    assert (S2, C2) == (S, C) and dz.is_contiguous(memory_format=CL) and dz.shape[1] == 128 and kprev.numel() >= 2 * C
    ws = _ws(call("mcl_dense_bn1_bwd_workspace_floats", S, C), x.device)
    if into_param_grads:
        dg, db = g1.grad, b1.grad
    else:
        dg = torch.empty(C, device=x.device, dtype=torch.float32)
        db = torch.empty(C, device=x.device, dtype=torch.float32)
    call("mcl_dense_bn1_dx_sums", dz, w16, C, px, ldx, S, g1, b1, mean,
         rstd, ws, dg, db, into_param_grads, kprev, have_prev, pg, ldg)
    return (None, None) if into_param_grads else (dg, db)


def dense_bn1_fix(buf: Tensor, gbuf: Tensor, c0: int, nc: int, mean: Tensor, rstd: Tensor, kacc: Tensor) -> None:
    px, S, _, ldx = _rows(buf)
    pg, S2, _, ldg = _rows(gbuf)
    assert S == S2
    call("mcl_dense_bn1_fix", px, ldx, pg, ldg, S, c0, nc, mean, rstd, kacc)


USE_BN1_SINGLE_PASS = True
BN1_SINGLE_PASS_MAX_MAP = 256

FUSED_BN1_WRW_MIN_PIXELS = 50000


def _bn1_wrw_ok(w_param: Tensor) -> bool:
    return (_direct_all(w_param) and w_param.grad.is_contiguous()
            and w_param.shape[0] == 128 and w_param.shape[2:] == (1, 1))


def dense_bn1_wrw(dz: Tensor, w16: Tensor, x: Tensor, g1: Tensor, b1: Tensor, mean: Tensor, rstd: Tensor, w_param: Tensor,
                  into_param_grads: bool):
    px, S, C, ldx = _rows(x)
    assert dz.is_contiguous(memory_format=CL) and dz.shape[1] == 128
    ws = _ws(call("mcl_wrw_workspace_floats", S, 128, C), x.device)
    if into_param_grads:
        dg, db = g1.grad, b1.grad
    else:
        dg = torch.empty(C, device=x.device, dtype=torch.float32)
        db = torch.empty(C, device=x.device, dtype=torch.float32)
    coef = torch.empty(2 * C, device=x.device, dtype=torch.float32)
    call("mcl_dense_bn1_wrw", dz, w16, C, px, ldx, S, g1, b1, mean, rstd, ws, w_param.grad, 1, dg, db, into_param_grads, coef)
    return (None, None, coef) if into_param_grads else (dg, db, coef)


def dense_bn1_dx(dz: Tensor, w16: Tensor, x: Tensor, g1: Tensor, b1: Tensor, mean: Tensor, rstd: Tensor, coef: Tensor,
                 gbuf: Tensor, window=None) -> None:
    px, S, C, ldx = _rows(x)
    pg, S2, C2, ldg = _rows(gbuf)
    assert (S2, C2) == (S, C)
    if window is None:
        call("mcl_dense_bn1_dx", dz, w16, C, px, ldx, S, g1, b1, mean, rstd, coef, pg, ldg)
    else:
        c0, nc = window
        call("mcl_dense_bn1_dx_window", dz, w16, C, c0, nc, px, ldx, S, g1, b1, mean, rstd, coef, pg, ldg)


def dense_bn1_dx_pair(A, B, x: Tensor, mean: Tensor, rstd: Tensor, gbuf: Tensor) -> None:
    dzA, wA, gA, bA, cA = A
    dzB, wB, gB, bB, cB = B
    px, S, C, ldx = _rows(x)
    pg, S2, C2, ldg = _rows(gbuf)
    assert (S2, C2) == (S, C) and wA.shape[1] >= C and wB.shape[1] == C
    call("mcl_dense_bn1_dx_pair", dzA, wA, wA.shape[1], gA, bA, cA, dzB, wB, gB, bB, cB, C, px, ldx, S, mean, rstd, pg, ldg)




def _c3_flat_kernel(W: int) -> bool:
    return W < 17 or W > 150


def dense_conv3x3_bwd(dy: Tensor, w16: Tensor, z: Tensor, g2: Tensor, b2: Tensor, m2: Tensor, r2: Tensor,
                      into_param_grads: bool, fix=None) -> Tuple[Tensor, Optional[Tensor], Optional[Tensor], Optional[Tensor]]:
    B, C, H, W = z.shape
    pd, S, Co, lddy = _rows(dy)
    assert C == 128 and Co == 32 and S == B * H * W and z.is_contiguous(memory_format=CL)
    ws = _ws(call("mcl_dense_conv3x3_bwd_workspace_floats", S), z.device)
    scratch = torch.empty_like(z, memory_format=CL)
    dz = torch.empty_like(z, memory_format=CL)
    if into_param_grads:
        dg, db = g2.grad, b2.grad
    else:
        dg = torch.empty(C, device=z.device, dtype=torch.float32)
        db = torch.empty(C, device=z.device, dtype=torch.float32)
    dyc = None
    if fix is not None:
        xf, fm, fr, fk = fix
        pxf, S2, C2, ldxf = _rows(xf)
        assert (S2, C2) == (S, 32) and fk.is_contiguous() and fk.numel() == 64
        dyc = torch.empty((B, 32, H, W), device=z.device, dtype=z.dtype, memory_format=CL)
        call("mcl_dense_conv3x3_bwd_fix", pd, lddy, S, H, W, w16, z, g2, b2, m2, r2,
             ws, dg, db, into_param_grads, scratch, dz, pxf, ldxf, fm, fr, fk, dyc)
    else:
        call("mcl_dense_conv3x3_bwd", pd, lddy, S, H, W, w16, z, g2, b2, m2, r2, ws, dg, db, into_param_grads, scratch, dz)
    return (dz, None, None, dyc) if into_param_grads else (dz, dg, db, dyc)




def dense_conv3x3_fwd(z: Tensor, g2: Tensor, b2: Tensor, m2: Tensor, r2: Tensor, w16: Tensor, out: Tensor, eps: float,
                      ymean: Optional[Tensor], yvar: Optional[Tensor], yrstd: Optional[Tensor]) -> None:
    B, C, H, W = z.shape
    po, S, Co, ldo = _rows(out)
    assert C == 128 and Co == 32 and z.is_contiguous(memory_format=CL) and S == B * H * W
    ws = _ws(call("mcl_dense_conv3x3_workspace_floats", S), z.device)
    call("mcl_dense_conv3x3_fwd", z, S, H, W, g2, b2, m2, r2, w16, po, ldo, ws, eps, ymean, yvar, yrstd)


def _grad_target_khwc(w_param: Tensor) -> Tuple[Tensor, bool]:
    g = w_param.grad
    if g.permute(0, 2, 3, 1).is_contiguous():
        return g, True
    co, ci, kh, kw = w_param.shape
    return torch.empty((co, kh, kw, ci), device=g.device, dtype=torch.float32), False


def _grad_finish_khwc(w_param: Tensor, tgt: Tensor, in_place: bool) -> None:
    if not in_place:
        w_param.grad.add_(tgt.permute(0, 3, 1, 2))


def dense_conv3x3_wrw(dy: Tensor, z: Tensor, g2: Tensor, b2: Tensor, m2: Tensor, r2: Tensor, w_param: Tensor) -> bool:
    if not _wrw3_direct_ok(w_param, z, dy):
        return False
    B, C, H, W = z.shape
    pd, S, Co, lddy = _rows(dy)
    assert Co == 32 and S == B * H * W
    tgt, in_place = _grad_target_khwc(w_param)
    ws = _ws(call("mcl_dense_conv3x3_wrw_workspace_floats", S), z.device)
    call("mcl_dense_conv3x3_wrw_det", pd, lddy, z, S, H, W, g2, b2, m2, r2, ws, tgt, in_place)
    _grad_finish_khwc(w_param, tgt, in_place)
    return True


def _wrw3_direct_ok(w_param: Tensor, z: Tensor, dy: Tensor) -> bool:
    return (_direct_all(w_param) and tuple(w_param.shape) == (32, 128, 3, 3)
            and dy.dtype == torch.bfloat16 and z.dtype == torch.bfloat16 and z.is_contiguous(memory_format=CL))


def _fused_3x3_ok(z: Tensor, w16: Tensor) -> bool:
    return (z.dtype == torch.bfloat16 and w16.dtype == torch.bfloat16
            and tuple(w16.shape) == (32, 128, 3, 3) and w16.permute(0, 2, 3, 1).is_contiguous()
            and z.shape[1] == 128 and z.shape[3] <= 150 and z.is_contiguous(memory_format=CL))


def _fused_1x1_ok(x: Tensor, w16: Tensor) -> bool:
    return (x.dtype == torch.bfloat16 and w16.dtype == torch.bfloat16 and w16.shape[0] == 128
            and w16.shape[1] % 8 == 0 and w16.shape[1] <= 1024 and w16.shape[2:] == (1, 1)
            and w16.permute(0, 2, 3, 1).is_contiguous())


def conv1x1_wrw(dz: Tensor, a: Tensor, w_param: Tensor, bn=None) -> Optional[Tensor]:
    pz, S, M, ldz = _rows(dz)
    pa, S2, N, lda = _rows(a)
    assert S == S2 and dz.dtype == a.dtype == torch.bfloat16
    if _direct_all(w_param) and w_param.grad.is_contiguous():
        tgt, ret = w_param.grad, None
    else:
        tgt = torch.zeros((M, N, 1, 1), device=dz.device, dtype=torch.float32)
        ret = tgt
    g_, b_, m_, r_ = bn if bn is not None else (None, None, None, None)
    ws = _ws(call("mcl_wrw_workspace_floats", S, min(M, 128), N), dz.device)
    call("mcl_conv1x1_wrw_det", pz, ldz, pa, lda, g_, b_, m_, r_, ws, tgt, 1, S, M, N)
    return ret


def _conv1x1_bwd(dz: Tensor, a: Tensor, w: Tensor, w_param: Tensor):
    return _conv_bwd(dz, a, w, w_param, 0)


def _same_order(a: Tensor, b: Tensor) -> bool:
    if a.shape != b.shape:
        return False
    sa = [s for s, n in zip(a.stride(), a.shape) if n > 1]
    sb = [s for s, n in zip(b.stride(), b.shape) if n > 1]
    dense = sorted(sa, reverse=True) and True
    return sa == sb and dense


def _wgrad(w: Tensor, dw: Tensor) -> Optional[Tensor]:
    if _direct_all(w) and _same_order(dw, w.grad) and dw.dtype in (
            torch.bfloat16, torch.float32):
        call("mcl_accum_into_f32", w.grad, dw, dw.numel(), _dt(dw))
        return None
    return dw.to(w.dtype)


_weight_provider = None

# ... 226 lines not shown
    arr = (C.c_void_p * len(ptrs))(*ptrs)
    nbytes = call("mcl_dense_block_fwd_workspace_bytes", B, L)
    ws = _ws((nbytes + 255 + 3) // 4 + 64, dev)
    base = (ws.data_ptr() + 255) & ~255
    from . import ops as _ops
    err = _ops.block_seam_error_flag(dev)
    px, S, C_, ld = _rows(buf)
    if ld != Ct:
        raise RuntimeError("dense_block_fwd_persistent: the concat buffer must be dense channels-last")
    call("mcl_dense_block_fwd", px, B, H, W, Ct, C0, L, arr, eps1, eps2, stats.mean,
         stats.var, stats.rstd, base, err, SEAM_MAX_SPINS, BLOCK_STAMPS)
    return zs


class _LayerPlan(NamedTuple):
    conv2: str
    conv1: str
    fix: str
    lanes: bool
    opens_pair: bool


def _plan_layer(l: int, cin: int, growth: int, B: int, H: int, W: int, fused1: bool, fused2: bool, w1_direct: bool,
                w2_direct: bool, kacc_live: bool, side_stream: bool, single_pass: bool, single_max_map: int,
                gram_min_pixels: int) -> _LayerPlan:
    conv2 = "own" if fused2 and w2_direct else "generic"
    if not fused1:
        conv1 = "generic"
    elif w1_direct and B * H * W >= gram_min_pixels:
        conv1 = "gram"
    elif single_pass and H * W <= single_max_map:
        conv1 = "single"
    else:
        conv1 = "two_pass"
    if not kacc_live:
        fix = "none"
    elif conv1 != "single":
        fix = "launch_all"
    elif growth == 32 and conv2 == "own" and _c3_flat_kernel(W):
        fix = "fold"
    else:
        fix = "launch_32"
    return _LayerPlan(conv2, conv1, fix, lanes=side_stream and conv1 != "generic" and conv2 == "own",
                      opens_pair=conv1 == "gram" and l >= 1 and growth == 32 and cin - growth >= 8)


class DenseBlockFn(torch.autograd.Function):

    @staticmethod
    def forward(ctx, x0, meta, *params):
        stats, eps1, eps2, growth, bn2_stats = meta[:5]
        prefilled = len(meta) > 5 and meta[5]
        ctx.first_block = (not prefilled) or (len(meta) > 6 and bool(meta[6]))
        L = len(params) // 6
        B, C0, H, W = x0.shape
        Ct = C0 + L * growth
        dev, dt = x0.device, x0.dtype
        pre = getattr(stats, "buf", None) if prefilled else None
        if (pre is not None and tuple(pre.shape) == (B, Ct, H, W) and pre.dtype == dt and x0.data_ptr() == pre.data_ptr()
                and x0.stride() == pre[:, :C0].stride()):
            buf, adopted = pre.detach(), True
        else:
            buf, adopted = torch.empty((B, Ct, H, W), device=dev, dtype=dt, memory_format=CL), False
            x0 = dense_cl(x0)
        if adopted:
            pass
        elif prefilled:
            buf[:, :C0].copy_(x0)
        else:
            bn_stats(x0, stats.mean[:C0], stats.var[:C0], stats.rstd[:C0], eps1[0], copy_out=buf[:, :C0])
        saved = []
        wcast = []
        kept_cols = {}
        ctx.persistent = False
        if _block_persistent_ok(buf, params, growth, L, C0, dt):
            wcast = [_weight(params[6 * l + k], dt) for l in range(L) for k in (2, 5)]
            zs = dense_block_fwd_persistent(buf, params, wcast, stats, bn2_stats, C0, L, eps1[0], eps2[0])
            for l in range(L):
                saved += [buf.new_empty(0), zs[l], buf.new_empty(0)]
            L_done = L
            ctx.persistent = True
        else:
            L_done = 0
        for l in range(L_done, L):
            g1, b1, w1, g2, b2, w2 = params[6 * l: 6 * l + 6]
            cin = C0 + l * growth
            w1c = _weight(w1, dt)
            m2, v2, r2 = bn2_stats[l]
            if _fused_1x1_ok(buf, w1c):
                a = None
                z = dense_conv1x1_fwd(buf[:, :cin], g1, b1, stats.mean[:cin], stats.rstd[:cin], w1c, eps2[l], m2, v2, r2)
            else:
                a = torch.empty((B, cin, H, W), device=dev, dtype=dt, memory_format=CL)
                bn_act_fwd(buf[:, :cin], g1, b1, stats.mean[:cin], stats.rstd[:cin], True, a)
                z = _conv1x1_fwd(a, w1c)
                bn_stats(z, m2, v2, r2, eps2[l])
            w2c = _weight(w2, dt)
            c1 = cin + growth
            if growth == 32 and _fused_3x3_ok(z, w2c):
                a2 = None
                dense_conv3x3_fwd(z, g2, b2, m2, r2, w2c, buf[:, cin:c1], eps1[min(l + 1, L - 1)],
                                  stats.mean[cin:c1], stats.var[cin:c1], stats.rstd[cin:c1])
            else:
                from . import conv_generic as cg
                a2 = torch.empty_like(z, memory_format=CL)
                bn_act_fwd(z, g2, b2, m2, r2, True, a2)
                _, cols2 = cg.conv_fwd(a2, w2c, 1, 1, out=buf[:, cin:c1], want_cols=True)
                kept_cols[l] = cols2
                bn_stats(buf[:, cin:c1], stats.mean[cin:c1], stats.var[cin:c1], stats.rstd[cin:c1], eps1[min(l + 1, L - 1)])
            saved += [a if a is not None else buf.new_empty(0), z, a2 if a2 is not None else buf.new_empty(0)]
            wcast += [w1c, w2c]
        ctx.save_for_backward(buf, *saved, *wcast)
        ctx.kept_cols = kept_cols
        ctx.params = params
        ctx.meta = (stats, growth, bn2_stats, L, C0)
        ctx.cap = None
        if CAPTURE_BLOCKS is not None:
            ctx.cap = {"buf": buf, "C0": C0, "growth": growth, "params": params, "wcast": wcast,
                       "mean": stats.mean, "rstd": stats.rstd, "var": stats.var, "z": saved[1::3], "bn2": bn2_stats}
            CAPTURE_BLOCKS.append(ctx.cap)
        return buf

    @staticmethod
    def backward(ctx, gbuf):
        stats, growth, bn2_stats, L, C0 = ctx.meta
        t = ctx.saved_tensors
        buf = t[0]
        dev = buf.device
        B, _, H, W = buf.shape
        params = ctx.params
        saved = t[1: 1 + 3 * L]
        wcast = t[1 + 3 * L:]
        if not gbuf.is_contiguous(memory_format=CL):
            gbuf = dense_cl(gbuf)
        if ctx.cap is not None:
            ctx.cap["gin"] = gbuf.clone(memory_format=CL)
            ctx.cap["dz"] = [None] * L
            ctx.cap["dyc"] = [None] * L
            ctx.cap["gbuf"] = gbuf
        grads = [None] * (6 * L)
        stamp(f"bwd block {buf.shape[2]}x{buf.shape[3]} start (main)")
        if getattr(ctx, "persistent", False) and _block_bwd_persistent_ok(buf, gbuf, params, L):
            zs = [saved[3 * l + 1] for l in range(L)]
            dzs, dycs = dense_block_bwd_persistent(buf, gbuf, params, wcast, zs, stats, bn2_stats, C0, L)
            if ctx.cap is not None:
                ctx.cap["dz"] = list(dzs)
                ctx.cap["dyc"] = list(dycs)
            gw1s = {}

            def _weight_grads():
                for l in range(L - 1, -1, -1):
                    g1, b1, w1, g2, b2, w2 = params[6 * l: 6 * l + 6]
                    cin = C0 + l * growth
                    m2, v2, r2 = bn2_stats[l]
                    ok = dense_conv3x3_wrw(dycs[l], zs[l], g2, b2, m2, r2, w2)
                    assert ok
                    gw1s[l] = conv1x1_wrw(dzs[l], buf[:, :cin], w1, bn=(g1, b1, stats.mean[:cin], stats.rstd[:cin]))
                if STAMPS:
                    stamp(f"bwd block {buf.shape[2]}x{buf.shape[3]} weight gradients done (side)")

            joins = buf.shape[0] * buf.shape[2] * buf.shape[3] >= JOIN_MIN_PIXELS or ctx.first_block
            lanes = USE_SIDE_STREAM and all(_direct_all(params[6 * l + 2]) and params[6 * l + 2].grad.is_contiguous()
                                            for l in range(L))
            _side_fork(dev, _weight_grads, (gbuf, buf, *dzs, *dycs, *zs), lanes=lanes, defer=True)
            if not lanes:
                for l in range(L):
                    grads[6 * l + 2] = gw1s[l]
            if STAMPS:
                stamp(f"bwd block {buf.shape[2]}x{buf.shape[3]} end (main)")
            if joins:
                _side_join(dev)
                stamp(f"bwd block {buf.shape[2]}x{buf.shape[3]} after join (main)")
            return (gbuf[:, :C0], None, *grads)
        kacc = None
        pair_a = None
        pair_cin = 0

        def flush_pair():
            nonlocal pair_a
            if pair_a is not None:
                dzA, wA, gA, bA, cA = pair_a
                dense_bn1_dx(dzA, wA, buf[:, :pair_cin], gA, bA, stats.mean[:pair_cin], stats.rstd[:pair_cin], cA,
                             gbuf[:, :pair_cin], window=(0, pair_cin - growth))
                pair_a = None

        def gram_dx(opens_pair, dz, w1c, g1, b1, cin, coef):
            nonlocal pair_a, pair_cin
            mine = (dz, w1c, g1, b1, coef)
            if pair_a is not None:
                dense_bn1_dx_pair(pair_a, mine, buf[:, :cin], stats.mean[:cin], stats.rstd[:cin], gbuf[:, :cin])
                pair_a = None
            elif opens_pair:
                dense_bn1_dx(dz, w1c, buf[:, :cin], g1, b1, stats.mean[:cin], stats.rstd[:cin], coef, gbuf[:, :cin],
                             window=(cin - growth, growth))
                pair_a, pair_cin = mine, cin
            else:
                dense_bn1_dx(dz, w1c, buf[:, :cin], g1, b1, stats.mean[:cin], stats.rstd[:cin], coef, gbuf[:, :cin])
        for l in range(L - 1, -1, -1):
            g1, b1, w1, g2, b2, w2 = params[6 * l: 6 * l + 6]
            a, z, a2 = saved[3 * l: 3 * l + 3]
            w1c, w2c = wcast[2 * l: 2 * l + 2]
            cin = C0 + l * growth
            c1 = cin + growth
            m2, v2, r2 = bn2_stats[l]
            x, gx, mean1, rstd1 = buf[:, :cin], gbuf[:, :cin], stats.mean[:cin], stats.rstd[:cin]
            dy_view = gbuf[:, cin:c1]
            d2 = _direct_all(g2, b2)
            d1 = _direct_all(g1, b1)
            fused1 = a.numel() == 0
            fused2 = a2.numel() == 0 and _fused_3x3_ok(z, w2c)
            plan = _plan_layer(l, cin, growth, B, H, W, fused1, fused2, fused1 and _bn1_wrw_ok(w1),
                               fused2 and _wrw3_direct_ok(w2, z, dy_view), kacc is not None, USE_SIDE_STREAM,
                               USE_BN1_SINGLE_PASS, BN1_SINGLE_PASS_MAX_MAP, FUSED_BN1_WRW_MIN_PIXELS)
            fold = None
            if plan.fix == "fold":
                fold = (buf[:, cin:c1], stats.mean[cin:c1], stats.rstd[cin:c1], kacc[cin:c1])
            elif plan.fix == "launch_32":
                dense_bn1_fix(buf, gbuf, cin, growth, stats.mean, stats.rstd, kacc)
            elif plan.fix == "launch_all":
                dense_bn1_fix(buf, gbuf, 0, c1, stats.mean, stats.rstd, kacc)
                kacc = None
            dw2 = None
            if plan.conv2 == "own":
                dz, dg2, db2, dyc = dense_conv3x3_bwd(dy_view, w2c, z, g2, b2, m2, r2, into_param_grads=d2, fix=fold)
            else:
                dyc = None
                if a2.numel() == 0:
                    a2 = torch.empty_like(z, memory_format=CL)
                    bn_act_fwd(z, g2, b2, m2, r2, True, a2)
                da2, dw2 = _conv_bwd(dy_view, a2, w2c, w2, 1, ctx.kept_cols.pop(l, None))
                dz = torch.empty_like(z, memory_format=CL)
                dg2, db2 = bn_act_bwd(dense_cl(da2), z, g2, b2, m2, r2, True, dz, False, into_param_grads=d2)
            dy_w = dyc if dyc is not None else dy_view
            if ctx.cap is not None:
                ctx.cap["dz"][l] = dz
                ctx.cap["dyc"][l] = dyc
            ev = _fork_event(dev) if plan.lanes else None
            if plan.conv1 != "gram":
                flush_pair()
            gw1 = None
            if plan.conv1 == "gram":
                dg1, db1, coef = dense_bn1_wrw(dz, w1c, x, g1, b1, mean1, rstd1, w1, into_param_grads=d1)
                gram_dx(plan.opens_pair, dz, w1c, g1, b1, cin, coef)
            elif plan.conv1 == "single":
                have_prev = kacc is not None
                if not have_prev:
                    kacc = torch.empty((buf.shape[1], 2), device=dev, dtype=torch.float32)
                dg1, db1 = dense_bn1_dx_sums(dz, w1c, x, g1, b1, mean1, rstd1, gx, kacc, have_prev, into_param_grads=d1)
            elif plan.conv1 == "two_pass":
                dg1, db1 = dense_bn1_bwd(dz, w1c, x, g1, b1, mean1, rstd1, gx, into_param_grads=d1)
            else:
                da, dw1 = _conv1x1_bwd(dz, a, w1c, w1)
                dg1, db1 = bn_act_bwd(da, x, g1, b1, mean1, rstd1, True, gx, True, into_param_grads=d1)
                gw1 = None if dw1 is None else _wgrad(w1, dw1)

            def weight_grads():
                if plan.conv2 == "own":
                    done = dense_conv3x3_wrw(dy_w, z, g2, b2, m2, r2, w2)
                    assert done
                if plan.conv1 in ("single", "two_pass"):
                    return conv1x1_wrw(dz, x, w1, bn=(g1, b1, mean1, rstd1))
                return gw1

            gw1 = _side_fork(dev, weight_grads, (dz, gbuf, z, buf, dy_w), lanes=plan.lanes, event=ev)
            grads[6 * l: 6 * l + 6] = [dg1, db1, gw1, dg2, db2, None if dw2 is None else _wgrad(w2, dw2)]
        flush_pair()
        if kacc is not None:
            dense_bn1_fix(buf, gbuf, 0, C0, stats.mean, stats.rstd, kacc)
        if STAMPS:
            stamp(f"bwd block {buf.shape[2]}x{buf.shape[3]} end (main)")
            if USE_SIDE_STREAM:
                with torch.cuda.stream(_side_stream(buf.device)):
                    stamp(f"bwd block {buf.shape[2]}x{buf.shape[3]} weight gradients done (side)")
        if buf.shape[0] * buf.shape[2] * buf.shape[3] >= JOIN_MIN_PIXELS or ctx.first_block:
            _side_join(buf.device)
            stamp(f"bwd block {buf.shape[2]}x{buf.shape[3]} after join (main)")
        return (gbuf[:, :C0], None, *grads)


def _bn_train(x: Tensor, bn: nn.BatchNorm2d, relu: bool, rec: _RunningStats) -> Tensor:
    C = x.shape[1]
    mean = torch.empty(C, device=x.device, dtype=torch.float32)
    var = torch.empty_like(mean)
    rstd = torch.empty_like(mean)
    x = dense_cl(x)
    bn_stats(x, mean, var, rstd, bn.eps)
    rec.add(bn, mean, var, x.numel() // C)
    return BNActFn.apply(x, bn.weight, bn.bias, mean, rstd, relu)


def dense_block(blk: nn.Module, x: Tensor, rec: _RunningStats, stats: Optional[_BlockStats] = None,
                force_join: bool = False) -> Tuple[Tensor, _BlockStats]:
    layers = list(blk.values())
    growth = layers[0].conv2.out_channels
    C0 = x.shape[1]
    Ct = C0 + len(layers) * growth
    prefilled = stats is not None
    if stats is None:
        stats = _BlockStats(Ct, x.device)
    bott = layers[0].conv1.out_channels
    bn2 = [tuple(torch.empty(bott, device=x.device, dtype=torch.float32) for _ in range(3)) for _ in layers]
    params = []
    for ly in layers:
        params += [ly.norm1.weight, ly.norm1.bias, ly.conv1.weight, ly.norm2.weight, ly.norm2.bias, ly.conv2.weight]
    meta = (stats, [ly.norm1.eps for ly in layers], [ly.norm2.eps for ly in layers], growth, bn2, prefilled, force_join)
    buf = DenseBlockFn.apply(x, meta, *params)
    n = x.shape[0] * x.shape[2] * x.shape[3]
# ... 530 lines not shown
```

mclstexp_amd/kernel_costs.py:

```python
from __future__ import annotations


def _conv1x1_wrw_det(a):
    S, M, N = a[11], a[12], a[13]
    return 2 * S * (M + N) + 4 * M * N


def _conv1x1_wrw_det_flops(a):
    return 2 * a[11] * a[12] * a[13]


def _conv3x3_wrw_det(a):
    S = a[3]
    return 2 * S * (32 + 128) + 4 * 32 * 1152


def _conv3x3_flops_S3(a):
    return 2 * a[3] * 32 * 1152


def _bn1_bwd(a):
    C, S = a[2], a[5]
    return 2 * S * (128 + C) + 2 * S * (128 + 3 * C)

# ... 76 lines not shown

def _bn1_dx_pair_flops(a):
    return 2 * 2 * a[14] * 128 * a[11]


def _bn1_dx_sums(a):
    C, S = a[2], a[5]
    return 2 * S * (128 + 3 * C)


def _bn1_fix(a):
    return 2 * a[4] * 3 * a[6]


def _adam_table(a):
    return 24 * a[3] * a[4]


def _adam_table_lazy(a):
    tables = 2 if a[4] else 1
    return tables * a[13] * a[9] * (24 + (4 if a[14] else 0))


def _block_fwd(a):
    B, HW, Ct, C0, L = a[1], a[2] * a[3], a[4], a[5], a[6]
    w = sum(128 * (C0 + 32 * l) * 2 for l in range(L)) + L * 32 * 1152 * 2
    return 2 * B * HW * C0 + L * 2 * B * HW * 128 + 2 * B * HW * 32 * L + w


def _block_fwd_flops(a):
    B, HW, C0, L = a[1], a[2] * a[3], a[5], a[6]
    return sum(2 * B * HW * (128 * (C0 + 32 * l) + 1152 * 32) for l in range(L))


def _block_bwd(a):
    B, HW, Ct, C0, L = a[2], a[3] * a[4], a[5], a[6], a[7]
    w = sum(128 * (C0 + 32 * l) * 2 for l in range(L)) + L * 32 * 1152 * 2
    return 2 * 2 * B * HW * Ct + 2 * B * HW * C0 + L * 2 * B * HW * (128 + 128 + 32) + w


def _block_bwd_flops(a):
    B, HW, C0, L = a[2], a[3] * a[4], a[6], a[7]
    return sum(2 * B * HW * (128 * (C0 + 32 * l) + 1152 * 32) for l in range(L))


def _adam(a):
    return 28 * a[4]


def _adam_shadow(a):
    return 30 * a[4]


def _zero(a):
    return 0


def _e(kernels, b, strict=None, flops=_zero, bound=None, unit=None):
    return {"kernels": kernels, "bytes": b, "strict": strict or b, "flops": flops, "bound": bound, "unit": unit}


TABLE = {
    "mcl_conv1x1_wrw_det": _e("wrw_partial_kernel + wrw_merge_kernel", _conv1x1_wrw_det, flops=_conv1x1_wrw_det_flops),
    "mcl_dense_conv3x3_wrw_det": _e("conv3x3_wrw_rows_kernel (56x56, 28x28 maps) / conv3x3_wrw_ky_kernel + wrw_merge_kernel",
                                    _conv3x3_wrw_det, flops=_conv3x3_flops_S3,
                                    bound="mfma/lds"),
    "mcl_dense_bn1_wrw": _e("wrw_partial_kernel<Gram> + wrw_merge_kernel", _bn1_wrw, flops=_bn1_wrw_flops),
    "mcl_dense_bn1_dx": _e("bn1_bwd_kernel<1> (one layer) / bn1_dx_pair_kernel (two consecutive layers' passes as one: "
                           "mcl_dense_bn1_dx_pair, preceded by the 32-channel mcl_dense_bn1_dx_window)", _bn1_dx, flops=_bn1_flops),
    "mcl_dense_bn1_dx_window": _e("bn1_bwd_kernel<1> on a 32-channel window", _bn1_dx_window, flops=_bn1_dx_window_flops,
                                  unit="mcl_dense_bn1_dx"),
    "mcl_dense_bn1_dx_pair": _e("bn1_dx_pair_kernel", _bn1_dx_pair, flops=_bn1_dx_pair_flops, unit="mcl_dense_bn1_dx"),
    "mcl_dense_bn1_dx_sums": _e("bn1_bwd_kernel<2> (single pass: dx data term + previous layer's mean terms + sums) + "
                                "bn1_bwd_finalize_kernel", _bn1_dx_sums, flops=_bn1_flops),
    "mcl_dense_bn1_fix": _e("bn1_fix_kernel", _bn1_fix, bound="latency"),
    "mcl_dense_bn1_bwd": _e("bn1_bwd_kernel<0> + bn1_bwd_finalize_kernel + bn1_bwd_kernel<1>", _bn1_bwd, _bn1_bwd_strict,
                            flops=lambda a: 2 * _bn1_flops(a)),
    "mcl_dense_conv3x3_bwd": _e("conv3x3_bwd_rows_kernel (56x56, 28x28 maps) / conv3x3_bwd_kernel (14x14, 7x7; with the "
                                "folded bn1_fix as mcl_dense_conv3x3_bwd_fix) + bn1_bwd_finalize_kernel + bn2_dz_kernel",
                                _conv3x3_bwd, _conv3x3_bwd_strict, flops=_conv3x3_flops_S2, bound="mfma/lds"),
    "mcl_dense_conv3x3_bwd_fix": _e("conv3x3_bwd_kernel (folded bn1_fix) + bn1_bwd_finalize_kernel + bn2_dz_kernel",
                                    _conv3x3_bwd_fix, _conv3x3_bwd_fix_strict, flops=_conv3x3_flops_S2, bound="mfma/lds",
                                    unit="mcl_dense_conv3x3_bwd"),
    "mcl_dense_conv1x1_fwd": _e("conv1x1_fwd_kernel + tile_stats_finalize_kernel", _conv1x1_fwd, flops=_conv1x1_fwd_flops),
    "mcl_dense_conv3x3_fwd": _e("conv3x3_fwd_rows_kernel + sums_finalize_kernel (56x56, 28x28 maps) / conv3x3_fwd_kernel + "
                                "tile_stats_finalize_kernel", _conv3x3_fwd, flops=_conv3x3_flops_S1, bound="mfma/lds"),
    "mcl_adam_table_step_dev": _e("adam_table_kernel", _adam_table, bound="hbm"),
    "mcl_dense_block_fwd": _e("dense_block_fwd_kernel (a whole 7x7 dense block forward: one persistent launch, in-launch batch-statistics "
                              "seams) + zero_words_kernel", _block_fwd, flops=_block_fwd_flops, bound="latency"),
    "mcl_dense_block_bwd": _e("dense_block_bwd_kernel (the block's data-gradient chain: one persistent launch) + zero_words_kernel",
                              _block_bwd, flops=_block_bwd_flops, bound="latency"),
    "mcl_adam_table_lazy": _e("adam_table_lazy_kernel (catch-up of gathered rows / update of the rows with a gradient)",
                              _adam_table_lazy, bound="latency"),
    "mcl_adam_step_dev": _e("adam_kernel", _adam, bound="hbm"),
    "mcl_adam_step_dev_shadow": _e("adam_kernel<shadow> (update + bf16 shadow of the parameters)", _adam_shadow, bound="hbm"),
}
```

Before: 12480 spots/s.

## Prepack 3x3 dense-conv weights per block and prefetch tiles in flat conv kernels

Adds a pack kernel that reorders each dense layer's 3x3 weights once per forward into the per-lane fragment layout. The flat (14x14, 7x7) forward and backward conv kernels can then load their B-operand registers with vector loads instead of many strided scalar gathers. The backward kernel also issues the next tile's z and dy/xfix slab loads into registers early, and the folded bn1 fix runs on those register copies. The cost is an extra pack launch and buffer per block, more register pressure, and templated kernel variants.

```diff
diff --git a/include/mclstexp_hip.h b/include/mclstexp_hip.h
--- a/include/mclstexp_hip.h
+++ b/include/mclstexp_hip.h
@@ -203,6 +203,12 @@
                           const float* mean, const float* rstd, const void* W2, void* out, int64_t ldo,
                           float* workspace, float eps, float* ymean, float* yvar, float* yrstd, mcl_stream_t stream);
 
+int mcl_dense_conv3x3_pack(const void* const* w2_ptrs, void* const* fwd_ptrs, void* const* bwd_ptrs, int32_t L, void* stream);
+int mcl_dense_conv3x3_fwd_packed(const void* z, int64_t S, int32_t H, int32_t W, const float* gamma, const float* beta,
+                                 const float* mean, const float* rstd, const void* W2, void* out, int64_t ldo,
+                                 float* workspace, float eps, float* ymean, float* yvar, float* yrstd, const void* W2p,
+                                 void* stream);
+
 int64_t mcl_dense_conv3x3_wrw_workspace_floats(int64_t S);
 int mcl_dense_conv3x3_wrw_det(const void* dy, int64_t lddy, const void* z, int64_t S, int32_t H, int32_t W,
                               const float* gamma, const float* beta, const float* mean, const float* rstd,
@@ -249,6 +255,16 @@
                               float* dgamma, float* dbeta, int32_t accumulate_params, void* g2, void* dz, const void* xfix,
                               int64_t ldxf, const float* fmean, const float* frstd, const float* fk, void* dyc,
                               mcl_stream_t stream);
+int mcl_dense_conv3x3_bwd_packed(const void* dy, int64_t lddy, int64_t S, int32_t H, int32_t W, const void* W2, const void* z,
+                                 const float* gamma, const float* beta, const float* mean, const float* rstd,
+                                 float* workspace, float* dgamma, float* dbeta, int32_t accumulate_params, void* g2, void* dz,
+                                 const void* W2p, void* stream);
+int mcl_dense_conv3x3_bwd_fix_packed(const void* dy, int64_t lddy, int64_t S, int32_t H, int32_t W, const void* W2,
+                                     const void* z, const float* gamma, const float* beta, const float* mean,
+                                     const float* rstd, float* workspace, float* dgamma, float* dbeta,
+                                     int32_t accumulate_params, void* g2, void* dz, const void* xfix, int64_t ldxf,
+                                     const float* fmean, const float* frstd, const float* fk, void* dyc, const void* W2p,
+                                     void* stream);
 
 int mcl_avgpool2_nhwc_bf16(const void* x, void* y, int32_t N, int32_t H, int32_t W, int32_t C, int32_t backward,
                            mcl_stream_t stream);
diff --git a/mclstexp_amd/_lib.py b/mclstexp_amd/_lib.py
--- a/mclstexp_amd/_lib.py
+++ b/mclstexp_amd/_lib.py
@@ -169,6 +169,12 @@
     "mcl_dense_bn1_fix": [c_p, c_l, c_p, c_l, c_l, c_i, c_i, c_p, c_p, c_p, c_s],
     "mcl_conv1x1_wrw_det": [c_p, c_l, c_p, c_l, c_p, c_p, c_p, c_p, c_p, c_p, c_i, c_l, c_i, c_i, c_s],
     "mcl_dense_conv3x3_fwd": [c_p, c_l, c_i, c_i, c_p, c_p, c_p, c_p, c_p, c_p, c_l, c_p, c_f, c_p, c_p, c_p, c_s],
+    "mcl_dense_conv3x3_pack": [c_p, c_p, c_p, c_i, c_p],
+    "mcl_dense_conv3x3_fwd_packed": [c_p, c_l, c_i, c_i, c_p, c_p, c_p, c_p, c_p, c_p, c_l, c_p, c_f, c_p, c_p, c_p, c_p, c_p],
+    "mcl_dense_conv3x3_bwd_packed": [c_p, c_l, c_l, c_i, c_i, c_p, c_p, c_p, c_p, c_p, c_p, c_p, c_p, c_p, c_i, c_p, c_p, c_p,
+                                     c_p],
+    "mcl_dense_conv3x3_bwd_fix_packed": [c_p, c_l, c_l, c_i, c_i, c_p, c_p, c_p, c_p, c_p, c_p, c_p, c_p, c_p, c_i, c_p, c_p,
+                                         c_p, c_l, c_p, c_p, c_p, c_p, c_p, c_p],
     "mcl_accum_into_f32": [c_p, c_p, c_l, c_i, c_s],
     "mcl_adam_step": [c_p, c_p, c_p, c_p, c_l, c_d, c_d, c_d, c_d, c_d, c_d, c_d, c_s],
     "mcl_adam_table_step": [c_p, c_p, c_p, c_i, c_i, c_p, c_p, c_l, c_d, c_d, c_d, c_d, c_d, c_d, c_d, c_s],
diff --git a/mclstexp_amd/csrc/dense_bwd.hip b/mclstexp_amd/csrc/dense_bwd.hip
--- a/mclstexp_amd/csrc/dense_bwd.hip
+++ b/mclstexp_amd/csrc/dense_bwd.hip
@@ -510,6 +510,22 @@
 
 constexpr int C3I = 128, C3O = 32, T3B = 128;
 
+__device__ __forceinline__ u32x4 fix_chunk(u32x4 g, u32x4 x, const float (&fka)[8], const float (&fkb)[8]) {
+  u32x4 o;
+#pragma unroll
+  for (int u = 0; u < 4; ++u) {
+    const float o_lo = __uint_as_float(g[u] << 16) - fmaf(fka[2 * u], __uint_as_float(x[u] << 16), fkb[2 * u]);
+    const float o_hi = __uint_as_float(g[u] & 0xFFFF0000u) -
+                       fmaf(fka[2 * u + 1], __uint_as_float(x[u] & 0xFFFF0000u), fkb[2 * u + 1]);
+    const f32x2 pv = {o_lo, o_hi};
+    o[u] = __builtin_bit_cast(unsigned, __builtin_convertvector(pv, bf16x2_t));
+  }
+  return o;
+}
+
+constexpr int SLAB_QB = 3;
+
+template <bool PACKED, bool FIX>
 __global__ __launch_bounds__(256, 1) void conv3x3_bwd_kernel(const bf16_t* __restrict__ dy, long long lddy, long long S,
                                                              int H, int W, const bf16_t* __restrict__ W2,
                                                              const bf16_t* __restrict__ z,
@@ -521,7 +537,8 @@
                                                              const bf16_t* __restrict__ xfix, long long ldxf,
                                                              const float* __restrict__ fmean,
                                                              const float* __restrict__ frstd,
-                                                             const float* __restrict__ fk, bf16_t* __restrict__ dyc) {
+                                                             const float* __restrict__ fk, bf16_t* __restrict__ dyc,
+                                                             const bf16_t* __restrict__ W2p) {
   extern __shared__ __attribute__((aligned(16))) unsigned char lds[];
   const int tid = threadIdx.x, lane = tid & 63, wave = tid >> 6;
   const int h = lane >> 5, l31 = lane & 31;
@@ -540,18 +557,59 @@
       zr[i] = p < Si ? *reinterpret_cast<const uint4*>(z + (long long)p * C3I + (tid & 15) * 8) : make_uint4(0u, 0u, 0u, 0u);
     }
   };
-  if ((int)blockIdx.x < ntile) load_z_tile(blockIdx.x);
+  u32x4 zq[8], dq[SLAB_QB], xq[SLAB_QB];
+  auto request_tile = [&](int tile) {
+    const int p0 = tile * T3B;
+#pragma unroll
+    for (int i = 0; i < 8; ++i) {
+      const int p = min(p0 + (tid >> 4) + 16 * i, Si - 1);
+      zq[i] = *reinterpret_cast<const u32x4*>(z + (long long)p * C3I + (tid & 15) * 8);
+    }
+  };
+  auto request_slab = [&](int tile) {
+    const int p0 = tile * T3B;
+#pragma unroll
+    for (int b = 0; b < SLAB_QB; ++b) {
+      const int q = tid + 256 * b;
+      const long long p = min(max(p0 - (W + 1) + (q >> 2), 0), Si - 1);
+      dq[b] = *reinterpret_cast<const u32x4*>(dy + p * lddy + (q & 3) * 8);
+      if constexpr (FIX) xq[b] = *reinterpret_cast<const u32x4*>(xfix + p * ldxf + (q & 3) * 8);
+    }
+  };
+  if constexpr (PACKED) request_tile(blockIdx.x);
+  else if ((int)blockIdx.x < ntile) load_z_tile(blockIdx.x);
   bf16x8 breg[18];
-#pragma unroll
-  for (int i = 0; i < 18; ++i) {
-    const int tap = i >> 1, co0 = 16 * (i & 1) + 8 * h;
-#pragma unroll
-    for (int j = 0; j < 8; ++j)
-      breg[i][j] = (short)W2[((long long)(co0 + j) * 9 + tap) * C3I + 32 * wave + l31];
+  if constexpr (PACKED) {
+#pragma unroll
+    for (int i = 0; i < 18; ++i)
+      breg[i] = *reinterpret_cast<const bf16x8*>(W2p + ((long long)(18 * wave + i) * 64 + lane) * 8);
+  } else {
+#pragma unroll
+    for (int i = 0; i < 18; ++i) {
+      const int tap = i >> 1, co0 = 16 * (i & 1) + 8 * h;
+#pragma unroll
+      for (int j = 0; j < 8; ++j)
+        breg[i][j] = (short)W2[((long long)(co0 + j) * 9 + tap) * C3I + 32 * wave + l31];
+    }
   }
   const int c = 32 * wave + l31;
   const float mu = mean[c], rs = rstd[c];
-  const float sc = gamma[c] * rs, sh = fmaf(-mu, sc, beta[c]);
+  const float gm = gamma[c], bt = beta[c];
+  float fk1[8], fk2[8], frs[8], fmn[8];
+  if constexpr (PACKED) {
+    if constexpr (FIX) {
+#pragma unroll
+      for (int e = 0; e < 8; ++e) {
+        const int cf = (tid & 3) * 8 + e;
+        fk1[e] = fk[2 * cf];
+        fk2[e] = fk[2 * cf + 1];
+        frs[e] = frstd[cf];
+        fmn[e] = fmean[cf];
+      }
+    }
+    request_slab(blockIdx.x);
+  }
+  const float sc = gm * rs, sh = fmaf(-mu, sc, bt);
   int abase[18];
 #pragma unroll
   for (int i = 0; i < 18; ++i) {
@@ -561,7 +619,15 @@
   }
   if (tid < 4) *reinterpret_cast<uint4*>(lds + zero_off + tid * 16) = make_uint4(0u, 0u, 0u, 0u);
   float fka[8], fkb[8];
-  if (xfix != nullptr) {
+  if constexpr (PACKED) {
+    if constexpr (FIX) {
+#pragma unroll
+      for (int e = 0; e < 8; ++e) {
+        fka[e] = fk2[e] * frs[e];
+        fkb[e] = fmaf(-fka[e], fmn[e], fk1[e]);
+      }
+    }
+  } else if (xfix != nullptr) {
 #pragma unroll
     for (int e = 0; e < 8; ++e) {
       const int cf = (tid & 3) * 8 + e;
@@ -571,8 +637,41 @@
     }
   }
 
-  for (int tile = blockIdx.x; tile < ntile; tile += gridDim.x) {
+  const int tile0 = blockIdx.x;
+  if constexpr (PACKED) __builtin_assume(tile0 < ntile);
+  for (int tile = tile0; tile < ntile; tile += gridDim.x) {
     const int p0 = tile * T3B;
+    if constexpr (PACKED) {
+      if (tile != (int)blockIdx.x) {
+        request_tile(tile);
+        request_slab(tile);
+      }
+      __syncthreads();
+      auto write_chunk = [&](int q, u32x4 g, u32x4 x) {
+        const int j = q >> 2, ch = q & 3;
+        const int p = p0 - (W + 1) + j;
+        const bool ok = p >= 0 && p < Si;
+        if constexpr (FIX) g = fix_chunk(g, x, fka, fkb);
+        const uint4 v = ok ? make_uint4(g[0], g[1], g[2], g[3]) : make_uint4(0u, 0u, 0u, 0u);
+        if constexpr (FIX)
+          if (ok && dyc != nullptr && j >= W + 1 && j < W + 1 + T3B) *reinterpret_cast<uint4*>(dyc + (long long)p * C3O + ch * 8) = v;
+        *reinterpret_cast<uint4*>(slab + j * 64 + ((ch ^ ((j >> 2) & 3)) << 4)) = v;
+      };
+#pragma unroll
+      for (int b = 0; b < SLAB_QB; ++b)
+        if (tid + 256 * b < nrow * 4) write_chunk(tid + 256 * b, dq[b], FIX ? xq[b] : dq[b]);
+      for (int q = tid + 256 * SLAB_QB; q < nrow * 4; q += 256) {
+        const long long pc = min(max(p0 - (W + 1) + (q >> 2), 0), Si - 1);
+        const u32x4 g = *reinterpret_cast<const u32x4*>(dy + pc * lddy + (q & 3) * 8);
+        u32x4 x = g;
+        if constexpr (FIX) x = *reinterpret_cast<const u32x4*>(xfix + pc * ldxf + (q & 3) * 8);
+        write_chunk(q, g, x);
+      }
+#pragma unroll
+      for (int i = 0; i < 8; ++i)
+        *reinterpret_cast<uint4*>(zt + ((tid >> 4) + 16 * i) * C3I + (tid & 15) * 8) =
+            p0 + (tid >> 4) + 16 * i < Si ? make_uint4(zq[i][0], zq[i][1], zq[i][2], zq[i][3]) : make_uint4(0u, 0u, 0u, 0u);
+    } else {
     if (tile != (int)blockIdx.x) load_z_tile(tile);
     __syncthreads();
     for (int q = tid; q < nrow * 4; q += 256) {
@@ -602,6 +701,7 @@
 #pragma unroll
     for (int i = 0; i < 8; ++i)
       *reinterpret_cast<uint4*>(zt + ((tid >> 4) + 16 * i) * C3I + (tid & 15) * 8) = zr[i];
+    }
     unsigned vmask[4];
 #pragma unroll
     for (int mb = 0; mb < 4; ++mb) {
@@ -1094,7 +1194,8 @@
 int conv3x3_bwd_impl(const void* dy, int64_t lddy, int64_t S, int32_t H, int32_t W, const void* W2, const void* z,
                      const float* gamma, const float* beta, const float* mean, const float* rstd, float* workspace,
                      float* dgamma, float* dbeta, int32_t accumulate_params, void* g2, void* dz, const void* xfix,
-                     int64_t ldxf, const float* fmean, const float* frstd, const float* fk, void* dyc, mcl_stream_t stream) {
+                     int64_t ldxf, const float* fmean, const float* frstd, const float* fk, void* dyc, const void* W2p,
+                     hipStream_t st) {
   MCL_CLEAR_ERROR();
   if (!dy || !W2 || !z || !gamma || !beta || !mean || !rstd || !workspace || !dgamma || !dbeta || !g2 || !dz || S <= 0 ||
       H <= 0 || W <= 0)
@@ -1109,7 +1210,7 @@
         (reinterpret_cast<uintptr_t>(dyc) & 15u))
       return MCL_EUNSUPPORTED;
   }
-  hipStream_t st = mcl_stream(stream);
+  if (reinterpret_cast<uintptr_t>(W2p) & 15u) return MCL_EUNSUPPORTED;
   float2* part = reinterpret_cast<float2*>(workspace);
   float* coef;
   if (bwd_rows_applicable(S, H, W)) {
@@ -1130,9 +1231,15 @@
     coef = workspace + (int64_t)ntile * 2 * C3I;
     const size_t lds_bytes = (size_t)T3B * 256 + (size_t)(T3B + 2 * W + 2) * 64 + 64;
     const int gcap = S >= 50000 ? 512 : 768;
-    hipLaunchKernelGGL(conv3x3_bwd_kernel, dim3(ntile < gcap ? ntile : gcap), dim3(256), lds_bytes, st, (const bf16_t*)dy,
-                       (long long)lddy, (long long)S, H, W, (const bf16_t*)W2, (const bf16_t*)z, gamma, beta, mean, rstd,
-                       (bf16_t*)g2, part, ntile, (const bf16_t*)xfix, (long long)ldxf, fmean, frstd, fk, (bf16_t*)dyc);
+#define MCL_LAUNCH(PK, FX)                                                                                                     \
+    hipLaunchKernelGGL((conv3x3_bwd_kernel<PK, FX>), dim3(ntile < gcap ? ntile : gcap), dim3(256), lds_bytes, st,               \
+                       (const bf16_t*)dy, (long long)lddy, (long long)S, H, W, (const bf16_t*)W2, (const bf16_t*)z, gamma, beta, \
+                       mean, rstd, (bf16_t*)g2, part, ntile, (const bf16_t*)xfix, (long long)ldxf, fmean, frstd, fk,            \
+                       (bf16_t*)dyc, (const bf16_t*)W2p)
+    if (!W2p) MCL_LAUNCH(false, false);
+    else if (xfix) MCL_LAUNCH(true, true);
+    else MCL_LAUNCH(true, false);
+#undef MCL_LAUNCH
     hipLaunchKernelGGL(bn1_bwd_finalize_kernel, dim3(C3I), dim3(256), 0, st, (const float2*)part, ntile, C3I,
                        (long long)S, dgamma, dbeta, coef, accumulate_params);
   }
@@ -1151,7 +1258,7 @@
                                      const float* rstd, float* workspace, float* dgamma, float* dbeta,
                                      int32_t accumulate_params, void* g2, void* dz, mcl_stream_t stream) {
   return conv3x3_bwd_impl(dy, lddy, S, H, W, W2, z, gamma, beta, mean, rstd, workspace, dgamma, dbeta, accumulate_params, g2,
-                          dz, nullptr, 0, nullptr, nullptr, nullptr, nullptr, stream);
+                          dz, nullptr, 0, nullptr, nullptr, nullptr, nullptr, nullptr, mcl_stream(stream));
 }
 
 extern "C" int mcl_dense_conv3x3_bwd_fix(const void* dy, int64_t lddy, int64_t S, int32_t H, int32_t W, const void* W2,
@@ -1162,5 +1269,24 @@
                                          mcl_stream_t stream) {
   if (!xfix) return MCL_EINVAL;
   return conv3x3_bwd_impl(dy, lddy, S, H, W, W2, z, gamma, beta, mean, rstd, workspace, dgamma, dbeta, accumulate_params, g2,
-                          dz, xfix, ldxf, fmean, frstd, fk, dyc, stream);
-}
+                          dz, xfix, ldxf, fmean, frstd, fk, dyc, nullptr, mcl_stream(stream));
+}
+
+extern "C" int mcl_dense_conv3x3_bwd_packed(const void* dy, int64_t lddy, int64_t S, int32_t H, int32_t W, const void* W2,
+                                            const void* z, const float* gamma, const float* beta, const float* mean,
+                                            const float* rstd, float* workspace, float* dgamma, float* dbeta,
+                                            int32_t accumulate_params, void* g2, void* dz, const void* W2p, void* stream) {
+  return conv3x3_bwd_impl(dy, lddy, S, H, W, W2, z, gamma, beta, mean, rstd, workspace, dgamma, dbeta, accumulate_params, g2,
+                          dz, nullptr, 0, nullptr, nullptr, nullptr, nullptr, W2p, reinterpret_cast<hipStream_t>(stream));
+}
+
+extern "C" int mcl_dense_conv3x3_bwd_fix_packed(const void* dy, int64_t lddy, int64_t S, int32_t H, int32_t W, const void* W2,
+                                                const void* z, const float* gamma, const float* beta, const float* mean,
+                                                const float* rstd, float* workspace, float* dgamma, float* dbeta,
+                                                int32_t accumulate_params, void* g2, void* dz, const void* xfix, int64_t ldxf,
+                                                const float* fmean, const float* frstd, const float* fk, void* dyc,
+                                                const void* W2p, void* stream) {
+  if (!xfix) return MCL_EINVAL;
+  return conv3x3_bwd_impl(dy, lddy, S, H, W, W2, z, gamma, beta, mean, rstd, workspace, dgamma, dbeta, accumulate_params, g2,
+                          dz, xfix, ldxf, fmean, frstd, fk, dyc, W2p, reinterpret_cast<hipStream_t>(stream));
+}
diff --git a/mclstexp_amd/csrc/dense_conv.hip b/mclstexp_amd/csrc/dense_conv.hip
--- a/mclstexp_amd/csrc/dense_conv.hip
+++ b/mclstexp_amd/csrc/dense_conv.hip
@@ -346,50 +346,115 @@
   }
 }
 
+template <int NB>
+__device__ __forceinline__ void slab_request(u32x4 (&v)[NB], const bf16_t* __restrict__ z, int p0, int Si, int W, int tid, int jb) {
+  const int cc = tid & 15;
+#pragma unroll
+  for (int i = 0; i < NB; ++i) {
+    const int p = p0 - (W + 1) + jb + 16 * i;
+    v[i] = *reinterpret_cast<const u32x4*>(z + (long long)min(max(p, 0), Si - 1) * C3_IN + cc * 8);
+  }
+}
+template <int NB>
+__device__ __forceinline__ void slab_write(unsigned char* lds, const u32x4 (&v)[NB], int p0, int Si, int W, int nrow, int tid,
+                                           int jb, const float (&sc)[8], const float (&sh)[8]) {
+  const int cc = tid & 15;
+#pragma unroll
+  for (int i = 0; i < NB; ++i) {
+    const int j = jb + 16 * i;
+    const int p = p0 - (W + 1) + j;
+    const bool ok = p >= 0 && p < Si;
+    if (j < nrow)
+      *reinterpret_cast<uint4*>(lds + j * 256 + ((cc ^ (j & 15)) << 4)) =
+          ok ? bn_relu_chunk(make_uint4(v[i][0], v[i][1], v[i][2], v[i][3]), sc, sh) : make_uint4(0u, 0u, 0u, 0u);
+  }
+}
+constexpr int SLAB_PA = 8, SLAB_PB = 3;
+
+template <bool PACKED>
 __global__ __launch_bounds__(256, 2) void conv3x3_fwd_kernel(const bf16_t* __restrict__ z, long long S, int H, int W,
                                                              const float* __restrict__ gamma,
                                                              const float* __restrict__ beta,
                                                              const float* __restrict__ mean,
                                                              const float* __restrict__ rstd,
                                                              const bf16_t* __restrict__ W2, bf16_t* __restrict__ out,
-                                                             long long ldo, float2* __restrict__ partial, int ntile) {
+                                                             long long ldo, float2* __restrict__ partial, int ntile,
+                                                             const bf16_t* __restrict__ W2p) {
   extern __shared__ __attribute__((aligned(16))) unsigned char lds[];
-  const int tid = threadIdx.x, lane = tid & 63, wave = tid >> 6;
+  const int tid = threadIdx.x, lane = tid & 63;
+  const int wave = PACKED ? __builtin_amdgcn_readfirstlane(tid >> 6) : tid >> 6;
   const int h = lane >> 5, l31 = lane & 31;
   const int nrow = T3 + 2 * W + 2;
   unsigned char* zero_row = lds + nrow * 256;
   const int Si = (int)S;
 
   bf16x8 breg[18];
-#pragma unroll
-  for (int i = 0; i < 18; ++i) {
-    const int kidx = 18 * wave + i;
-    breg[i] = *reinterpret_cast<const bf16x8*>(W2 + ((long long)l31 * 9 + (kidx >> 3)) * C3_IN + 16 * (kidx & 7) + 8 * h);
+  u32x4 za[SLAB_PA], zb[SLAB_PB];
+  if constexpr (PACKED) {
+    const bf16_t* __restrict__ wf = W2p + (long long)wave * (18 * 512);
+    const unsigned lo = (unsigned)lane * 8u;
+#pragma unroll
+    for (int i = 0; i < 18; ++i) breg[i] = *reinterpret_cast<const bf16x8*>(wf + i * 512 + lo);
+  } else {
+#pragma unroll
+    for (int i = 0; i < 18; ++i) {
+      const int kidx = 18 * wave + i;
+      breg[i] = *reinterpret_cast<const bf16x8*>(W2 + ((long long)l31 * 9 + (kidx >> 3)) * C3_IN + 16 * (kidx & 7) + 8 * h);
+    }
   }
   float sc[8], sh[8];
   {
     const int cc = tid & 15;
+    float gm[8], bt[8], mn[8], rs[8];
 #pragma unroll
     for (int i = 0; i < 8; ++i) {
       const int c = cc * 8 + i;
-      sc[i] = gamma[c] * rstd[c];
-      sh[i] = fmaf(-mean[c], sc[i], beta[c]);
+      gm[i] = gamma[c];
+      rs[i] = rstd[c];
+      mn[i] = mean[c];
+      bt[i] = beta[c];
+    }
+    if constexpr (PACKED) {
+      slab_request<SLAB_PA>(za, z, (int)blockIdx.x * T3, Si, W, tid, tid >> 4);
+      __builtin_amdgcn_sched_barrier(0);
+    }
+#pragma unroll
+    for (int i = 0; i < 8; ++i) {
+      sc[i] = gm[i] * rs[i];
+      sh[i] = fmaf(-mn[i], sc[i], bt[i]);
     }
   }
   int abase[18], tapk[18];
-#pragma unroll
-  for (int i = 0; i < 18; ++i) {
-    const int kidx = 18 * wave + i, tap = kidx >> 3, kk = kidx & 7;
-    const int row = l31 + (tap / 3) * W + (tap % 3);
-    abase[i] = row * 256 + (((2 * kk + h) ^ (row & 15)) << 4);
-    tapk[i] = tap;
-  }
-  for (int tile = blockIdx.x; tile < ntile; tile += gridDim.x) {
+  auto fragment_offsets = [&](int ln) {
+#pragma unroll
+    for (int i = 0; i < 18; ++i) {
+      const int kidx = 18 * wave + i, tap = kidx >> 3, kk = kidx & 7;
+      const int row = (ln & 31) + (tap / 3) * W + (tap % 3);
+      abase[i] = row * 256 + (((2 * kk + (ln >> 5)) ^ (row & 15)) << 4);
+      tapk[i] = tap;
+    }
+  };
+  if constexpr (!PACKED) fragment_offsets(lane);
+  const int tile0 = blockIdx.x;
+  if constexpr (PACKED) __builtin_assume(tile0 < ntile);
+  for (int tile = tile0; tile < ntile; tile += gridDim.x) {
   const int p0 = tile * T3;
   __syncthreads();
 
-  stage_slab<SLAB_NB>(lds, z, p0, S, W, nrow, tid, sc, sh);
+  if constexpr (PACKED) {
+    if (tile != (int)blockIdx.x) slab_request<SLAB_PA>(za, z, p0, Si, W, tid, tid >> 4);
+    slab_write<SLAB_PA>(lds, za, p0, Si, W, nrow, tid, tid >> 4, sc, sh);
+    slab_request<SLAB_PB>(zb, z, p0, Si, W, tid, (tid >> 4) + 16 * SLAB_PA);
+    slab_write<SLAB_PB>(lds, zb, p0, Si, W, nrow, tid, (tid >> 4) + 16 * SLAB_PA, sc, sh);
+    for (int jb = (tid >> 4) + 16 * (SLAB_PA + SLAB_PB); jb < nrow; jb += 16 * SLAB_PA) {
+      slab_request<SLAB_PA>(za, z, p0, Si, W, tid, jb);
+      slab_write<SLAB_PA>(lds, za, p0, Si, W, nrow, tid, jb, sc, sh);
+    }
+  } else {
+    stage_slab<SLAB_NB>(lds, z, p0, S, W, nrow, tid, sc, sh);
+  }
   if (tid < 16) *reinterpret_cast<uint4*>(zero_row + tid * 16) = make_uint4(0u, 0u, 0u, 0u);
+  if constexpr (PACKED) fragment_offsets(opaque_lane(lane));
 
   unsigned vmask[4];
 #pragma unroll
@@ -435,7 +500,8 @@
       red[(wave * T3 + px) * C3_OUT + l31] = acc[mb][r];
     }
   __syncthreads();
-  const int px = tid >> 1, c0 = (tid & 1) * 16;
+  const int te = PACKED ? opaque_lane(tid) : tid;
+  const int px = te >> 1, c0 = (te & 1) * 16;
   const long long p = (long long)p0 + px;
   float v[16];
 #pragma unroll
@@ -465,7 +531,7 @@
   }
   __syncthreads();
   {
-    const int c = tid & 31, g = tid >> 5;
+    const int c = te & 31, g = te >> 5;
     const float ks = rv[c];
     const int nvalid = min(T3, Si - p0);
     float s1 = 0.0f, s2 = 0.0f;
@@ -481,15 +547,15 @@
     grp[(g * 32 + c) * 2] = s1;
     grp[(g * 32 + c) * 2 + 1] = s2;
     __syncthreads();
-    if (tid < 32) {
+    if (te < 32) {
       float a = 0.0f, b = 0.0f;
 #pragma unroll
       for (int gg = 0; gg < 8; ++gg) {
-        a += grp[(gg * 32 + tid) * 2];
-        b += grp[(gg * 32 + tid) * 2 + 1];
+        a += grp[(gg * 32 + te) * 2];
+        b += grp[(gg * 32 + te) * 2 + 1];
       }
       const float n = (float)nvalid;
-      partial[(long long)tid * ntile + tile] = make_float2(fmaf(n, rv[tid], a), b - a * a / n);
+      partial[(long long)te * ntile + tile] = make_float2(fmaf(n, rv[te], a), b - a * a / n);
     }
   }
   }
@@ -501,10 +567,58 @@
   return flat > rows ? flat : rows;
 }
 
-extern "C" int mcl_dense_conv3x3_fwd(const void* z, int64_t S, int32_t H, int32_t W, const float* gamma,
-                                     const float* beta, const float* mean, const float* rstd, const void* W2, void* out,
-                                     int64_t ldo, float* workspace, float eps, float* ymean, float* yvar, float* yrstd,
-                                     mcl_stream_t stream) {
+constexpr int PACK3_MAXL = 64, PACK3_PIECES = 72 * 64;
+struct Pack3Args {
+  const bf16_t* w2[PACK3_MAXL];
+  bf16_t* fwd[PACK3_MAXL];
+  bf16_t* bwd[PACK3_MAXL];
+};
+__global__ __launch_bounds__(256) void pack_w2_kernel(Pack3Args p) {
+  const int l = blockIdx.y;
+  const int q = blockIdx.x * 256 + threadIdx.x;
+  const bf16_t* __restrict__ w2 = p.w2[l];
+  if (q < PACK3_PIECES) {
+    const int lane = q & 63, f = q >> 6, l31 = lane & 31, h = lane >> 5;
+    *reinterpret_cast<uint4*>(p.fwd[l] + (long long)q * 8) =
+        *reinterpret_cast<const uint4*>(w2 + ((long long)l31 * 9 + (f >> 3)) * C3_IN + 16 * (f & 7) + 8 * h);
+  } else if (q < 2 * PACK3_PIECES) {
+    const int r = q - PACK3_PIECES, lane = r & 63, i = (r >> 6) % 18, wave = (r >> 6) / 18;
+    const int tap = i >> 1, co0 = 16 * (i & 1) + 8 * (lane >> 5), ci = 32 * wave + (lane & 31);
+    unsigned v[8];
+#pragma unroll
+    for (int j = 0; j < 8; ++j) v[j] = w2[((long long)(co0 + j) * 9 + tap) * C3_IN + ci];
+    *reinterpret_cast<uint4*>(p.bwd[l] + (long long)r * 8) =
+        make_uint4(v[0] | (v[1] << 16), v[2] | (v[3] << 16), v[4] | (v[5] << 16), v[6] | (v[7] << 16));
+  }
+}
+
+extern "C" int mcl_dense_conv3x3_pack(const void* const* w2_ptrs, void* const* fwd_ptrs, void* const* bwd_ptrs, int32_t L,
+                                      void* stream) {
+  MCL_CLEAR_ERROR();
+  if (!w2_ptrs || !fwd_ptrs || !bwd_ptrs || L <= 0) return MCL_EINVAL;
+  for (int l = 0; l < L; ++l)
+    if (!w2_ptrs[l] || !fwd_ptrs[l] || !bwd_ptrs[l] || (reinterpret_cast<uintptr_t>(w2_ptrs[l]) & 15u) ||
+        (reinterpret_cast<uintptr_t>(fwd_ptrs[l]) & 15u) || (reinterpret_cast<uintptr_t>(bwd_ptrs[l]) & 15u))
+      return MCL_EINVAL;
+  for (int l0 = 0; l0 < L; l0 += PACK3_MAXL) {
+    const int n = L - l0 < PACK3_MAXL ? L - l0 : PACK3_MAXL;
+    Pack3Args p;
+    for (int l = 0; l < PACK3_MAXL; ++l) {
+      const int k = l0 + (l < n ? l : 0);
+      p.w2[l] = (const bf16_t*)w2_ptrs[k];
+      p.fwd[l] = (bf16_t*)fwd_ptrs[k];
+      p.bwd[l] = (bf16_t*)bwd_ptrs[k];
+    }
+    hipLaunchKernelGGL(pack_w2_kernel, dim3(2 * PACK3_PIECES / 256, n), dim3(256), 0, reinterpret_cast<hipStream_t>(stream), p);
+  }
+  MCL_CHECK_LAUNCH();
+  return MCL_OK;
+}
+
+namespace {
+int conv3x3_fwd_impl(const void* z, int64_t S, int32_t H, int32_t W, const float* gamma, const float* beta, const float* mean,
+                     const float* rstd, const void* W2, const void* W2p, void* out, int64_t ldo, float* workspace, float eps,
+                     float* ymean, float* yvar, float* yrstd, hipStream_t st) {
   MCL_CLEAR_ERROR();
   if (!z || !gamma || !beta || !mean || !rstd || !W2 || !out || !workspace || S <= 0 || H <= 0 || W <= 0)
     return MCL_EINVAL;
@@ -515,7 +629,7 @@
     return MCL_EUNSUPPORTED;
   if (mcl_conv3x3_rows_applicable(S, H, W)) {
     const int rc = mcl_launch_conv3x3_fwd_rows(z, S, H, W, gamma, beta, mean, rstd, W2, out, ldo, workspace, eps, ymean,
-                                               yvar, yrstd, mcl_stream(stream));
+                                               yvar, yrstd, st);
     if (rc != 0) return rc;
     MCL_CHECK_LAUNCH();
     return MCL_OK;
@@ -523,20 +637,45 @@
   const int ntile = (int)((S + T3 - 1) / T3);
   size_t lds_bytes = (size_t)(T3 + 2 * W + 2) * 256 + 256;
   if (lds_bytes < 4 * T3 * C3_OUT * 4) lds_bytes = 4 * T3 * C3_OUT * 4;
-  hipStream_t st = mcl_stream(stream);
   static mcl_device_once attr_once;
   if (auto attr_guard = attr_once.first()) {
-    (void)hipFuncSetAttribute(reinterpret_cast<const void*>(conv3x3_fwd_kernel),
+    (void)hipFuncSetAttribute(reinterpret_cast<const void*>(conv3x3_fwd_kernel<false>),
                               hipFuncAttributeMaxDynamicSharedMemorySize, 112 * 1024);
+    (void)hipFuncSetAttribute(reinterpret_cast<const void*>(conv3x3_fwd_kernel<true>),
+                              hipFuncAttributeMaxDynamicSharedMemorySize, 112 * 1024);
   }
   float2* part = reinterpret_cast<float2*>(workspace);
-  hipLaunchKernelGGL(conv3x3_fwd_kernel, dim3(ntile < 512 ? ntile : 512), dim3(256), lds_bytes, st, (const bf16_t*)z, (long long)S, H, W,
-                     gamma, beta, mean, rstd, (const bf16_t*)W2, (bf16_t*)out, (long long)ldo, part, ntile);
+  if (W2p)
+    hipLaunchKernelGGL(conv3x3_fwd_kernel<true>, dim3(ntile < 512 ? ntile : 512), dim3(256), lds_bytes, st, (const bf16_t*)z,
+                       (long long)S, H, W, gamma, beta, mean, rstd, (const bf16_t*)W2, (bf16_t*)out, (long long)ldo, part, ntile,
+                       (const bf16_t*)W2p);
+  else
+    hipLaunchKernelGGL(conv3x3_fwd_kernel<false>, dim3(ntile < 512 ? ntile : 512), dim3(256), lds_bytes, st, (const bf16_t*)z,
+                       (long long)S, H, W, gamma, beta, mean, rstd, (const bf16_t*)W2, (bf16_t*)out, (long long)ldo, part, ntile,
+                       (const bf16_t*)nullptr);
   if (want_stats)
     hipLaunchKernelGGL(tile_stats_finalize_kernel, dim3(C3_OUT), dim3(256), 0, st, (const float2*)part, ntile,
                        C3_OUT, (long long)S, T3, eps, ymean, yvar, yrstd);
   MCL_CHECK_LAUNCH();
   return MCL_OK;
+}
+}
+
+extern "C" int mcl_dense_conv3x3_fwd(const void* z, int64_t S, int32_t H, int32_t W, const float* gamma,
+                                     const float* beta, const float* mean, const float* rstd, const void* W2, void* out,
+                                     int64_t ldo, float* workspace, float eps, float* ymean, float* yvar, float* yrstd,
+                                     mcl_stream_t stream) {
+  return conv3x3_fwd_impl(z, S, H, W, gamma, beta, mean, rstd, W2, nullptr, out, ldo, workspace, eps, ymean, yvar, yrstd,
+                          mcl_stream(stream));
+}
+
+extern "C" int mcl_dense_conv3x3_fwd_packed(const void* z, int64_t S, int32_t H, int32_t W, const float* gamma,
+                                            const float* beta, const float* mean, const float* rstd, const void* W2,
+                                            void* out, int64_t ldo, float* workspace, float eps, float* ymean, float* yvar,
+                                            float* yrstd, const void* W2p, void* stream) {
+  if (reinterpret_cast<uintptr_t>(W2p) & 15u) return MCL_EUNSUPPORTED;
+  return conv3x3_fwd_impl(z, S, H, W, gamma, beta, mean, rstd, W2, W2p, out, ldo, workspace, eps, ymean, yvar, yrstd,
+                          reinterpret_cast<hipStream_t>(stream));
 }
 
 namespace {
diff --git a/mclstexp_amd/densenet_fused.py b/mclstexp_amd/densenet_fused.py
--- a/mclstexp_amd/densenet_fused.py
+++ b/mclstexp_amd/densenet_fused.py
@@ -358,8 +358,29 @@
     return W < 17 or W > 150
 
 
+PACKED_W2_ELEMS = 32 * 9 * 128
+USE_PACKED_W2 = os.environ.get("MCL_PACKED_W2", "1") != "0"
+
+
+def _pack_w2_ok(w16: Tensor) -> bool:
+    return (w16.is_cuda and w16.dtype == torch.bfloat16 and tuple(w16.shape) == (32, 128, 3, 3)
+            and w16.permute(0, 2, 3, 1).is_contiguous() and w16.data_ptr() % 16 == 0)
+
+
+def dense_conv3x3_pack(w16s) -> List[Tuple[Tensor, Tensor]]:
+    import ctypes as C
+    L = len(w16s)
+    assert L > 0 and all(_pack_w2_ok(w) for w in w16s)
+    buf = torch.empty((L, 2, PACKED_W2_ELEMS), device=w16s[0].device, dtype=torch.bfloat16)
+    vp = C.c_void_p * L
+    call("mcl_dense_conv3x3_pack", vp(*[w.data_ptr() for w in w16s]), vp(*[buf[l, 0].data_ptr() for l in range(L)]),
+         vp(*[buf[l, 1].data_ptr() for l in range(L)]), L, current_stream())
+    return [(buf[l, 0], buf[l, 1]) for l in range(L)]
+
+
 def dense_conv3x3_bwd(dy: Tensor, w16: Tensor, z: Tensor, g2: Tensor, b2: Tensor, m2: Tensor, r2: Tensor,
-                      into_param_grads: bool, fix=None) -> Tuple[Tensor, Optional[Tensor], Optional[Tensor], Optional[Tensor]]:
+                      into_param_grads: bool, fix=None,
+                      packed: Optional[Tensor] = None) -> Tuple[Tensor, Optional[Tensor], Optional[Tensor], Optional[Tensor]]:
     B, C, H, W = z.shape
     pd, S, Co, lddy = _rows(dy)
     assert C == 128 and Co == 32 and S == B * H * W and z.is_contiguous(memory_format=CL)
@@ -377,8 +398,15 @@
         pxf, S2, C2, ldxf = _rows(xf)
         assert (S2, C2) == (S, 32) and fk.is_contiguous() and fk.numel() == 64
         dyc = torch.empty((B, 32, H, W), device=z.device, dtype=z.dtype, memory_format=CL)
-        call("mcl_dense_conv3x3_bwd_fix", pd, lddy, S, H, W, w16, z, g2, b2, m2, r2,
-             ws, dg, db, into_param_grads, scratch, dz, pxf, ldxf, fm, fr, fk, dyc)
+        if packed is not None:
+            call("mcl_dense_conv3x3_bwd_fix_packed", pd, lddy, S, H, W, w16, z, g2, b2, m2, r2,
+                 ws, dg, db, into_param_grads, scratch, dz, pxf, ldxf, fm, fr, fk, dyc, packed, current_stream())
+        else:
+            call("mcl_dense_conv3x3_bwd_fix", pd, lddy, S, H, W, w16, z, g2, b2, m2, r2,
+                 ws, dg, db, into_param_grads, scratch, dz, pxf, ldxf, fm, fr, fk, dyc)
+    elif packed is not None:
+        call("mcl_dense_conv3x3_bwd_packed", pd, lddy, S, H, W, w16, z, g2, b2, m2, r2, ws, dg, db, into_param_grads, scratch,
+             dz, packed, current_stream())
     else:
         call("mcl_dense_conv3x3_bwd", pd, lddy, S, H, W, w16, z, g2, b2, m2, r2, ws, dg, db, into_param_grads, scratch, dz)
     return (dz, None, None, dyc) if into_param_grads else (dz, dg, db, dyc)
@@ -387,12 +415,17 @@
 
 
 def dense_conv3x3_fwd(z: Tensor, g2: Tensor, b2: Tensor, m2: Tensor, r2: Tensor, w16: Tensor, out: Tensor, eps: float,
-                      ymean: Optional[Tensor], yvar: Optional[Tensor], yrstd: Optional[Tensor]) -> None:
+                      ymean: Optional[Tensor], yvar: Optional[Tensor], yrstd: Optional[Tensor],
+                      packed: Optional[Tensor] = None) -> None:
     B, C, H, W = z.shape
     po, S, Co, ldo = _rows(out)
     assert C == 128 and Co == 32 and z.is_contiguous(memory_format=CL) and S == B * H * W
     ws = _ws(call("mcl_dense_conv3x3_workspace_floats", S), z.device)
-    call("mcl_dense_conv3x3_fwd", z, S, H, W, g2, b2, m2, r2, w16, po, ldo, ws, eps, ymean, yvar, yrstd)
+    if packed is not None:
+        call("mcl_dense_conv3x3_fwd_packed", z, S, H, W, g2, b2, m2, r2, w16, po, ldo, ws, eps, ymean, yvar, yrstd, packed,
+             current_stream())
+    else:
+        call("mcl_dense_conv3x3_fwd", z, S, H, W, g2, b2, m2, r2, w16, po, ldo, ws, eps, ymean, yvar, yrstd)
 
 
 def _grad_target_khwc(w_param: Tensor) -> Tuple[Tensor, bool]:
@@ -785,6 +818,13 @@
             ctx.persistent = True
         else:
             L_done = 0
+        w2cs, packs = {}, {}
+        if USE_PACKED_W2 and growth == 32 and dt == torch.bfloat16 and _c3_flat_kernel(W) and x0.is_cuda and L_done < L:
+            w2cs = {l: _weight(params[6 * l + 5], dt) for l in range(L_done, L)}
+            ok = [l for l in w2cs if _pack_w2_ok(w2cs[l])]
+            if ok:
+                packs = dict(zip(ok, dense_conv3x3_pack([w2cs[l] for l in ok])))
+        ctx.w2_packs = {l: fb[1] for l, fb in packs.items()}
         for l in range(L_done, L):
             g1, b1, w1, g2, b2, w2 = params[6 * l: 6 * l + 6]
             cin = C0 + l * growth
@@ -798,12 +838,13 @@
                 bn_act_fwd(buf[:, :cin], g1, b1, stats.mean[:cin], stats.rstd[:cin], True, a)
                 z = _conv1x1_fwd(a, w1c)
                 bn_stats(z, m2, v2, r2, eps2[l])
-            w2c = _weight(w2, dt)
+            w2c = w2cs[l] if l in w2cs else _weight(w2, dt)
             c1 = cin + growth
             if growth == 32 and _fused_3x3_ok(z, w2c):
                 a2 = None
                 dense_conv3x3_fwd(z, g2, b2, m2, r2, w2c, buf[:, cin:c1], eps1[min(l + 1, L - 1)],
-                                  stats.mean[cin:c1], stats.var[cin:c1], stats.rstd[cin:c1])
+                                  stats.mean[cin:c1], stats.var[cin:c1], stats.rstd[cin:c1],
+                                  packed=packs[l][0] if l in packs else None)
             else:
                 from . import conv_generic as cg
                 a2 = torch.empty_like(z, memory_format=CL)
@@ -925,7 +966,8 @@
                 kacc = None
             dw2 = None
             if plan.conv2 == "own":
-                dz, dg2, db2, dyc = dense_conv3x3_bwd(dy_view, w2c, z, g2, b2, m2, r2, into_param_grads=d2, fix=fold)
+                dz, dg2, db2, dyc = dense_conv3x3_bwd(dy_view, w2c, z, g2, b2, m2, r2, into_param_grads=d2, fix=fold,
+                                                      packed=ctx.w2_packs.get(l))
             else:
                 dyc = None
                 if a2.numel() == 0:
diff --git a/mclstexp_amd/kernel_costs.py b/mclstexp_amd/kernel_costs.py
--- a/mclstexp_amd/kernel_costs.py
+++ b/mclstexp_amd/kernel_costs.py
@@ -182,6 +182,14 @@
     "mcl_dense_conv3x3_bwd_fix": _e("conv3x3_bwd_kernel (folded bn1_fix) + bn1_bwd_finalize_kernel + bn2_dz_kernel",
                                     _conv3x3_bwd_fix, _conv3x3_bwd_fix_strict, flops=_conv3x3_flops_S2, bound="mfma/lds",
                                     unit="mcl_dense_conv3x3_bwd"),
+    "mcl_dense_conv3x3_bwd_packed": _e("conv3x3_bwd_kernel<packed> + bn1_bwd_finalize_kernel + bn2_dz_kernel",
+                                       _conv3x3_bwd, _conv3x3_bwd_strict, flops=_conv3x3_flops_S2, bound="mfma/lds",
+                                       unit="mcl_dense_conv3x3_bwd"),
+    "mcl_dense_conv3x3_bwd_fix_packed": _e("conv3x3_bwd_kernel<packed> (folded bn1_fix) + bn1_bwd_finalize_kernel + bn2_dz_kernel",
+                                           _conv3x3_bwd_fix, _conv3x3_bwd_fix_strict, flops=_conv3x3_flops_S2, bound="mfma/lds",
+                                           unit="mcl_dense_conv3x3_bwd"),
+    "mcl_dense_conv3x3_fwd_packed": _e("conv3x3_fwd_kernel<packed> + tile_stats_finalize_kernel", _conv3x3_fwd,
+                                       flops=_conv3x3_flops_S1, bound="mfma/lds", unit="mcl_dense_conv3x3_fwd"),
     "mcl_dense_conv1x1_fwd": _e("conv1x1_fwd_kernel + tile_stats_finalize_kernel", _conv1x1_fwd, flops=_conv1x1_fwd_flops),
     "mcl_dense_conv3x3_fwd": _e("conv3x3_fwd_rows_kernel + sums_finalize_kernel (56x56, 28x28 maps) / conv3x3_fwd_kernel + "
                                 "tile_stats_finalize_kernel", _conv3x3_fwd, flops=_conv3x3_flops_S1, bound="mfma/lds"),
```

Result: no change. 12560 spots/s (median of 6 runs) (+0.6%).
